# ysong1231/SimRank

Hardware: AMD Instinct MI355X
Metric: simrank_iterations_per_sec (higher is better)
Workload: dtype f32

## Files before the change

### simrank_amd/csrc/api.hip

```cpp
#include <algorithm>
#include <chrono>
#include <cstring>
#include <mutex>
#include <unordered_map>
#include <string>
#include <thread>
#include <vector>

#include "common.h"

namespace simrank {

static thread_local char g_err[512] = "";

void set_error(const char* fmt, ...) {
    va_list ap;
    va_start(ap, fmt);
    vsnprintf(g_err, sizeof(g_err), fmt, ap);
    va_end(ap);
}

Tuning& tuning() {
    static Tuning t;
    return t;
// ... 747 lines not shown
extern "C" {

int simrank_graph_destroy(simrank_graph* g) {
    if (!g) return SIMRANK_OK;
    plan_free(g->rowptr);
    plan_free(g->col);
    plan_free(g->col16);
    plan_free(g->rowscale);
    plan_free(g->t_rowptr);
    plan_free(g->t_col);
    plan_free(g->t_pos);
    plan_free(g->ev_hubidx);
    plan_free(g->ev_hub_image);
#ifndef SIMRANK_HOST_ONLY
    if (g->ev_hub_ready) (void)hipEventDestroy((hipEvent_t)g->ev_hub_ready);
#endif
    plan_free(g->tile_row0);
    plan_free(g->sym_map);
    free_dense_plan(g->dense);
    free_fused_plan(g->fused);
#ifdef SIMRANK_EXPERIMENT_FUSED2
    free_fused2_plan(g->fused2);
#endif
    delete g;
    return SIMRANK_OK;
}

int simrank_graph_set_dense_terms(simrank_graph* g, int32_t terms) {
    SR_REQUIRE(g, "graph is NULL");
    SR_REQUIRE(terms == 1 || terms == 3, "dense terms must be 3 (exact) or 1 (fp16 operand)");
    g->tun.dense_terms = terms;
    return SIMRANK_OK;
}

int simrank_graph_shape(const simrank_graph* g, int64_t* n_rows, int64_t* n_cols, int64_t* nnz) {
    SR_REQUIRE(g, "graph is NULL");
    if (n_rows) *n_rows = g->n_rows;
    if (n_cols) *n_cols = g->n_cols;
    if (nnz) *nnz = g->nnz;
    return SIMRANK_OK;
}

int simrank_set_tuning(const char* key, int64_t value) {
    SR_REQUIRE(key, "key is NULL");
    std::lock_guard<std::mutex> lock(tuning_mutex());
    Tuning& t = tuning();
    if (!strcmp(key, "panel")) {
        SR_REQUIRE(value == 0 || value == 16 || value == 32 || value == 64 || value == 128 ||
                       value == 256,
                   "panel must be 0, 16, 32, 64, 128 or 256");
        t.panel = value;
    } else if (!strcmp(key, "xcd_map")) {
        t.xcd_map = value ? 1 : 0;
    } else if (!strcmp(key, "tile")) {
        SR_REQUIRE(value == 0 || value == 16 || value == 32 || value == 64, "tile must be 0, 16, 32 or 64");
        t.tile = value;
    } else if (!strcmp(key, "huge")) {
        SR_REQUIRE(value >= 64 && value <= (1 << 30), "huge must be >= 64");
        t.huge = value;
    } else if (!strcmp(key, "triangle")) {
        t.triangle = value ? 1 : 0;
    } else if (!strcmp(key, "stream_nt")) {
        t.stream_nt = value ? 1 : 0;
    } else if (!strcmp(key, "balance")) {
        SR_REQUIRE(value >= 0 && value <= 1024, "balance must be 0 (uniform tiles) .. 1024");
        t.balance = value;
    } else if (!strcmp(key, "dense_min")) {
        SR_REQUIRE(value >= 0 && value <= 128, "dense_min must be 0 (off) .. 128");
        t.dense_min = value;
    } else if (!strcmp(key, "probe_mask")) {
        SR_REQUIRE(value < 0 || getenv("SIMRANK_ENABLE_PROBES"),
                   "probe knobs give WRONG results (measurement only): set SIMRANK_ENABLE_PROBES=1 to use them");
        t.probe_mask = value < 0 ? -1 : value;
    } else if (!strcmp(key, "dense_terms")) {
        SR_REQUIRE(value == 1 || value == 3, "dense_terms must be 3 (exact) or 1 (fp16 operand)");
        t.dense_terms = value;
    } else if (!strcmp(key, "probe_flags")) {
        SR_REQUIRE(value == 0 || getenv("SIMRANK_ENABLE_PROBES"),
                   "probe knobs give WRONG results (measurement only): set SIMRANK_ENABLE_PROBES=1 to use them");
        t.probe_flags = value & 63;
    } else if (!strcmp(key, "addr32")) {
        t.addr32 = value ? 1 : 0;
    } else if (!strcmp(key, "lean")) {
        SR_REQUIRE(value == 0 || value == 1, "lean must be 0 or 1");
        t.lean = value;
    } else if (!strcmp(key, "ids16")) {
        t.ids16 = value ? 1 : 0;
    } else if (!strcmp(key, "sym_desc")) {
        t.sym_desc = value ? 1 : 0;
    } else if (!strcmp(key, "dense_sym")) {
        t.dense_sym = value < 0 ? -1 : (value ? 1 : 0);
    } else if (!strcmp(key, "fuse")) {
#ifdef SIMRANK_EXPERIMENT_FUSED2
        SR_REQUIRE(value >= 0 && value <= 2, "fuse must be 0 (two launches), 1 (one launch) or 2 (one persistent launch)");
#else
        SR_REQUIRE(value == 0 || value == 1, "fuse must be 0 (two launches) or 1 (one launch)");
#endif
        t.fuse = value;
    } else if (!strcmp(key, "ev_hub")) {
        SR_REQUIRE(value >= 0 && value <= 1000, "ev_hub must be 0 (off) .. 1000 (thousandths of the row count)");
        t.ev_hub = value;
    } else if (!strcmp(key, "fuse_min")) {
        SR_REQUIRE(value == 0 || (value >= 2 && value <= 128), "fuse_min must be 2 .. 128, or 0 (quads that pay)");
        t.fuse_min = value;
    } else if (!strcmp(key, "fuse_pays")) {
        SR_REQUIRE(value >= -1 && value <= 8192, "fuse_pays must be -1 (automatic) .. 8192");
        t.fuse_pays = value;
    } else if (!strcmp(key, "fuse_unit")) {
        SR_REQUIRE(value >= 4 && value <= (1 << 20), "fuse_unit must be >= 4");
        t.fuse_unit = value;
    } else if (!strcmp(key, "fuse_store")) {
        SR_REQUIRE(value >= 0 && value <= 3, "fuse_store must be 0 .. 3");
        t.fuse_store = value;
    } else if (!strcmp(key, "fuse_meta_nt")) {
        t.fuse_meta_nt = value ? 1 : 0;
    } else if (!strcmp(key, "fuse_order")) {
        SR_REQUIRE(value >= 0 && value <= 64, "fuse_order must be 0 .. 64");
        t.fuse_order = value;
    } else if (!strcmp(key, "fuse_max_rows")) {
        SR_REQUIRE(value >= 0, "fuse_max_rows must be >= 0");
        t.fuse_max_rows = value;
    } else if (!strcmp(key, "fuse_rows")) {
        SR_REQUIRE(value >= 64 && value <= (int64_t(1) << 40), "fuse_rows must be >= 64");
        t.fuse_rows = value;
    } else if (!strcmp(key, "ev_tri")) {
        t.ev_tri = value ? 1 : 0;
    } else if (!strcmp(key, "fuse_shards")) {
        t.fuse_shards = value ? 1 : 0;
    } else if (!strcmp(key, "fuse_cap")) {
        SR_REQUIRE(value >= 1000 && value <= (int64_t(1) << 40), "fuse_cap must be >= 1000");
        t.fuse_cap = value;
    } else if (!strcmp(key, "fuse_wgs")) {
        SR_REQUIRE(value >= 1 && value <= 8, "fuse_wgs must be 1 .. 8");
        t.fuse_wgs = value;
    } else if (!strcmp(key, "fuse_group")) {
        SR_REQUIRE(value >= 1 && value <= 4, "fuse_group must be 1 .. 4");
        t.fuse_group = value;
    } else if (!strcmp(key, "fuse_sym")) {
        SR_REQUIRE(value >= -1 && value <= 1, "fuse_sym must be -1 (automatic), 0 or 1");
        t.fuse_sym = value;
    } else if (!strcmp(key, "fuse_steps")) {
        SR_REQUIRE(value >= -1 && value <= (1 << 20), "fuse_steps must be >= 0, or -1 (by the operand's size)");
        t.fuse_steps = value;
    } else if (!strcmp(key, "fuse_dens")) {
        SR_REQUIRE(value >= 0 && value <= (1 << 20), "fuse_dens must be >= 0");
        t.fuse_dens = value;
    } else if (!strcmp(key, "dense_cols")) {
        SR_REQUIRE(value >= 1 && value <= (1 << 20), "dense_cols must be >= 1");
        t.dense_cols = value;
    } else if (!strcmp(key, "restrict_support")) {
        SR_REQUIRE(value >= -1 && value <= 1, "restrict_support must be -1 (automatic), 0 or 1");
        t.restrict_support = value;
    } else if (!strcmp(key, "leg1_skip")) {
        t.leg1_skip = value ? 1 : 0;
    } else if (!strcmp(key, "leg1_order")) {
        SR_REQUIRE(value >= -1 && value <= 1, "leg1_order must be -1 (by the graph's size), 0 or 1");
        t.leg1_order = value;
    } else {
        SR_REQUIRE(false, "unknown tuning key '%s'", key);
    }
    return SIMRANK_OK;
}

int simrank_get_tuning(const char* key, int64_t* value) {
    SR_REQUIRE(key && value, "NULL argument");
    const Tuning t = tuning_snapshot();
    if (!strcmp(key, "panel")) *value = t.panel;
    else if (!strcmp(key, "xcd_map")) *value = t.xcd_map;
    else if (!strcmp(key, "stream_nt")) *value = t.stream_nt;
    else if (!strcmp(key, "tile")) *value = t.tile;
    else if (!strcmp(key, "triangle")) *value = t.triangle;
    else if (!strcmp(key, "huge")) *value = t.huge;
    else if (!strcmp(key, "balance")) *value = t.balance;
    else if (!strcmp(key, "dense_min")) *value = t.dense_min;
    else if (!strcmp(key, "dense_cols")) *value = t.dense_cols;
    else if (!strcmp(key, "dense_sym")) *value = t.dense_sym;
    else if (!strcmp(key, "fuse")) *value = t.fuse;
    else if (!strcmp(key, "ev_hub")) *value = t.ev_hub;
    else if (!strcmp(key, "fuse_min")) *value = t.fuse_min;
    else if (!strcmp(key, "fuse_pays")) *value = t.fuse_pays;
    else if (!strcmp(key, "fuse_steps")) *value = t.fuse_steps;
    else if (!strcmp(key, "fuse_dens")) *value = t.fuse_dens;
    else if (!strcmp(key, "fuse_unit")) *value = t.fuse_unit;
    else if (!strcmp(key, "fuse_group")) *value = t.fuse_group;
    else if (!strcmp(key, "fuse_sym")) *value = t.fuse_sym;
    else if (!strcmp(key, "fuse_cap")) *value = t.fuse_cap;
    else if (!strcmp(key, "fuse_shards")) *value = t.fuse_shards;
    else if (!strcmp(key, "ev_tri")) *value = t.ev_tri;
    else if (!strcmp(key, "fuse_rows")) *value = t.fuse_rows;
    else if (!strcmp(key, "fuse_wgs")) *value = t.fuse_wgs;
    else if (!strcmp(key, "fuse_max_rows")) *value = t.fuse_max_rows;
    else if (!strcmp(key, "fuse_order")) *value = t.fuse_order;
    else if (!strcmp(key, "fuse_store")) *value = t.fuse_store;
    else if (!strcmp(key, "fuse_meta_nt")) *value = t.fuse_meta_nt;
    else if (!strcmp(key, "sym_desc")) *value = t.sym_desc;
    else if (!strcmp(key, "ids16")) *value = t.ids16;
    else if (!strcmp(key, "lean")) *value = t.lean;
    else if (!strcmp(key, "addr32")) *value = t.addr32;
    else if (!strcmp(key, "probe_flags")) *value = t.probe_flags;
    else if (!strcmp(key, "dense_terms")) *value = t.dense_terms;
    else if (!strcmp(key, "probe_mask")) *value = t.probe_mask;
    else if (!strcmp(key, "restrict_support")) *value = t.restrict_support;
    else if (!strcmp(key, "leg1_skip")) *value = t.leg1_skip;
    else if (!strcmp(key, "leg1_order")) *value = t.leg1_order;
    else SR_REQUIRE(false, "unknown tuning key '%s'", key);
    return SIMRANK_OK;
}

int simrank_graph_get(const simrank_graph* g, const char* key, int64_t* value) {
    SR_REQUIRE(g && key && value, "NULL argument");
    if (!strcmp(key, "fused_ids16")) *value = g->fused ? g->fused->ids16 : -1;
    else if (!strcmp(key, "gather_ids16")) *value = (g->col16 && g->tun.ids16) ? 1 : 0;
    else SR_REQUIRE(false, "unknown graph key '%s'", key);
    return SIMRANK_OK;
}

}
```

### simrank_amd/csrc/common.h

```cpp
#pragma once
#include <hip/hip_runtime.h>

#include <cstdarg>
#include <atomic>
#include <cstdint>
#include <cstdio>
#include <cstdlib>
#include <cstring>
#include <functional>
#include <vector>

#include "simrank_hip.h"

namespace simrank {

void set_error(const char* fmt, ...);

#define SR_HIP(call)                                                                   \
    do {                                                                               \
        hipError_t e_ = (call);                                                        \
        if (e_ != hipSuccess) {                                                        \
            ::simrank::set_error("%s failed: %s (%s:%d)", #call, hipGetErrorString(e_), \
                                 __FILE__, __LINE__);                                  \
            return SIMRANK_ERR_HIP;                                                    \
        }                                                                              \
    } while (0)

#define SR_REQUIRE(cond, ...)                 \
    do {                                      \
        if (!(cond)) {                        \
            ::simrank::set_error(__VA_ARGS__); \
            return SIMRANK_ERR_INVALID;       \
        }                                     \
    } while (0)

struct Tuning {
    int64_t panel = 0;
    int64_t xcd_map = 1;
    int64_t stream_nt = 1;
    int64_t tile = 0;
    int64_t huge = 512;
    int64_t triangle = 1;
    int64_t balance = 2;
    int64_t dense_min = 4;
    int64_t dense_cols = 128;
    int64_t dense_terms = 3;
    int64_t probe_mask = -1;
    int64_t probe_flags = 0;
    int64_t addr32 = 1;
    int64_t lean = 1;
    int64_t ids16 = 1;
    int64_t sym_desc = 1;
    int64_t ev_tri = 1;
    int64_t ev_hub = 14;
    int64_t fuse = 1;
    int64_t fuse_min = 0;
    int64_t fuse_pays = -1;
    int64_t fuse_steps = -1;
    int64_t fuse_dens = 0;
    int64_t fuse_unit = 48;
    int64_t fuse_rows = 8192;
    int64_t fuse_store = 1;
    int64_t fuse_meta_nt = 0;
    int64_t fuse_order = 0;
    int64_t fuse_max_rows = 1 << 20;
    int64_t fuse_cap = 40000;
    int64_t fuse_wgs = 4;
    int64_t fuse_shards = 1;
    int64_t fuse_group = 3;
    int64_t fuse_sym = -1;
    int64_t leg1_skip = 1;
    int64_t leg1_order = -1;
    int64_t dense_lazy = 0;
    int64_t dense_sym = -1;
    int64_t restrict_support = -1;
};
inline int32_t restrict_choice(const Tuning& t, int64_t live, int64_t total) {
    return t.restrict_support < 0 ? (2 * live < total ? 1 : 0) : int32_t(t.restrict_support != 0);
}
Tuning& tuning();
Tuning tuning_snapshot();


#ifdef SIMRANK_HOST_ONLY
inline hipError_t plan_alloc(void** p, size_t bytes) {
    *p = malloc(bytes ? bytes : 1);
    return *p ? hipSuccess : hipErrorOutOfMemory;
}
inline hipError_t plan_upload(void* d, const void* h, size_t bytes) { memcpy(d, h, bytes); return hipSuccess; }
inline hipError_t plan_download(void* h, const void* d, size_t bytes) { memcpy(h, d, bytes); return hipSuccess; }
inline void plan_free(void* p) { free(p); }
#else
int pool_alloc(void** dptr, size_t bytes);
int pool_free(void* ptr);
inline hipError_t plan_alloc(void** p, size_t bytes) {
    const int rc = pool_alloc(p, bytes);
    return rc == SIMRANK_OK ? hipSuccess : (rc == SIMRANK_ERR_ALLOC ? hipErrorOutOfMemory : hipErrorUnknown);
}
inline hipError_t plan_upload(void* d, const void* h, size_t bytes) { return hipMemcpy(d, h, bytes, hipMemcpyHostToDevice); }
inline hipError_t plan_download(void* h, const void* d, size_t bytes) { return hipMemcpy(h, d, bytes, hipMemcpyDeviceToHost); }
inline void plan_free(void* p) { (void)pool_free(p); }
#endif

int graph_create_with(const Tuning& tun, int64_t n_rows, int64_t n_cols, int64_t nnz, const int32_t* rowptr,
                      const int32_t* col, const float* rowscale, simrank_graph** out,
                      const std::function<int(simrank_graph*)>* after_base = nullptr);

int pool_alloc(void** dptr, size_t bytes);
int pool_free(void* ptr);
void pool_trim(int device);
void pool_stats(int device, int64_t* cached_bytes, int64_t* cached_blocks, int64_t* limit_bytes);
void handback_release_slabs(int device);
int rows_to_host(const void* S, int64_t rows_pad, int64_t n, const int32_t* inv_dev, const int32_t* rows, int32_t n_rows,
                 float* dst, int64_t ld, int elem, float scale, hipStream_t stream);
inline hipError_t pool_hip_alloc(void** p, size_t bytes) {
    const int rc = pool_alloc(p, bytes);
    return rc == SIMRANK_OK ? hipSuccess : (rc == SIMRANK_ERR_ALLOC ? hipErrorOutOfMemory : hipErrorUnknown);
}

int identity_leg1_blocked(const simrank_graph* g, float* Tt, int64_t t_rows_pad, void* stream);
int identity_leg1_blocked_h16(const simrank_graph* g, uint16_t* Tt, int64_t t_rows_pad, float scale, void* stream);

struct PlanPrep {
    std::vector<int32_t> ord, inv;
    std::vector<int32_t> rp, cl;
    std::vector<float> rs;
    bool asym = false;
    std::vector<int32_t> first_block;
};
constexpr int32_t kLeg1Never = 0x7FFFFFFF;
void first_block_table(int64_t n, const int32_t* rp, const int32_t* cl, std::vector<int32_t>& first_block);
struct BiPlanPrep {
    std::vector<int32_t> rowptr21, col21;
    std::vector<int32_t> ord[2], inv[2];
    std::vector<int32_t> rp[2], cl[2];
    std::vector<float> rs[2];
    bool asym = false;
};
int plan_prepare(int64_t n, int64_t nnz, const int32_t* rowptr, const int32_t* col, const float* rowscale,
                 const simrank_plan_options* opt, PlanPrep* out);
int shard_prepare(int64_t n, int64_t nnz, const int32_t* rowptr, const int32_t* col, const float* rowscale,
                  const float* apriori, int64_t ld_apriori, bool reorder, int32_t deal, PlanPrep* out, bool allow_asym = false);
int shard_biplan_prepare(int64_t n1, int64_t n2, int64_t nnz, const int32_t* rowptr12, const int32_t* col12,
                         const float* rowscale1, const float* rowscale2, const simrank_biplan_options* opt, int32_t deal1,
                         int32_t deal2, BiPlanPrep* out, bool allow_asym = false);
bool prior_symmetric(const float* a, int64_t ld, int64_t n);
int biplan_prepare(int64_t n1, int64_t n2, int64_t nnz, const int32_t* rowptr12, const int32_t* col12,
                   const float* rowscale1, const float* rowscale2, const simrank_biplan_options* opt, BiPlanPrep* out);

inline int64_t fuse_min_steps(const Tuning& t, int64_t K) {
    return t.fuse_steps >= 0 ? t.fuse_steps : (K * 128 > (int64_t(4) << 20) ? 8 : 20);
}

constexpr int64_t kSpeculateBelow = 16384;

inline hipStream_t as_stream(void* s) { return reinterpret_cast<hipStream_t>(s); }
inline bool aligned16(const void* p) { return (reinterpret_cast<uintptr_t>(p) & 15u) == 0; }

}


struct simrank_dense_plan {
    int32_t n_units = 0;
    int32_t n_slabs = 0;
    int32_t n_blocks_dense = 0;
    int64_t total_k = 0;
    int64_t nnz_covered = 0;
    int32_t* unit_row0 = nullptr;
    int32_t* unit_slab = nullptr;
    int32_t* unit_kofs = nullptr;
    int32_t* dcols = nullptr;
    uint4* afrag = nullptr;
    int32_t* block_slab0 = nullptr;
    int32_t* block_nslab = nullptr;
    int64_t r_nnz = 0;
    int32_t r_max_row = 0;
    int32_t* r_rowptr = nullptr;
    int32_t* r_col = nullptr;
    uint16_t* r_col16 = nullptr;
    int32_t* r_tile_row0 = nullptr;
    int32_t r_n_tiles = 0;
    int32_t* r_sym_map = nullptr;
    int32_t r_sym_blocks = 0;
    float* part = nullptr;
    size_t part_cap = 0;
};

struct simrank_fused_plan {
    int32_t n_units = 0;
    int32_t n_blocks = 0;
    int32_t ids16 = 0;
    int64_t n_quads = 0;
    int64_t n_steps = 0;
    int64_t nnz_covered = 0;
    int64_t r_nnz = 0;
    int32_t* units = nullptr;
    int32_t n_pslots = 0, n_cslots = 0;
    float* partials = nullptr;
    int32_t* tickets = nullptr;
    int32_t cap_panels = 0;
    uint16_t* dcols16 = nullptr;
    int32_t* dcols32 = nullptr;
    uint4* abits = nullptr;
    int2* gmeta = nullptr;
    uint16_t* sids16 = nullptr;
    int32_t* sids32 = nullptr;
    std::vector<int32_t> unit_last;
};

#ifdef SIMRANK_EXPERIMENT_FUSED2
struct simrank_fused2_plan {
    int32_t n_items = 0;
    int32_t n_blocks = 0;
    int32_t ids16 = 0;
    int32_t cap_panels = 0;
    int64_t n_quads = 0, n_steps = 0, nnz_covered = 0, r_nnz = 0;
    int32_t* items = nullptr;
    int32_t n_pslots = 0, n_cslots = 0;
    float* partials = nullptr;
    int32_t* tickets = nullptr;
    uint32_t* heads = nullptr;
    uint16_t* dcols16 = nullptr;
    int32_t* dcols32 = nullptr;
    uint4* abits = nullptr;
    int2* gmeta = nullptr;
    uint16_t* sids16 = nullptr;
    int32_t* sids32 = nullptr;
};
#endif

namespace simrank {
constexpr int kFB = 128;
constexpr int kSub = 4;
void free_fused_plan(simrank_fused_plan* p);
int build_fused_plan(simrank_graph* g, const int32_t* rowptr, const int32_t* col, const float* rowscale);
int launch_fused_trans(const simrank_graph* g, const float* X, int64_t x_rows_pad, int64_t L, float* Y,
                       int64_t y_rows_pad, hipStream_t st, const int32_t* first_block = nullptr);
void fused_leg1_counts(const simrank_graph* g, int64_t L, const int32_t* first_block_host, int64_t* units, int64_t* skipped);
int spmm_blocked_is_triangle(const simrank_graph* g, const float* X, int64_t x_rows_pad, int64_t n_cols_x, float* Y,
                             int64_t y_rows_pad, const simrank_epilogue* ep, bool* triangle);
int spmm_blocked_leg1(const simrank_graph* g, const float* X, int64_t x_rows_pad, int64_t n_cols_x, float* Y,
                      int64_t y_rows_pad, const int32_t* first_block, bool* skipping, void* stream);
bool fused_sym_applies(const simrank_graph* g, int64_t x_rows_pad, int64_t L, int64_t y_rows_pad);
int launch_fused_sym(const simrank_graph* g, const float* X, int64_t x_rows_pad, int64_t L, float* Y, int64_t y_rows_pad,
                     float coef, float lbd, double eps, const uint8_t* ev, const float* ap, const float* prev,
                     unsigned long long* n_changed, int32_t set_diag, int32_t count_any, hipStream_t st);
bool fused_rowmajor_fits(const simrank_graph* g, const float* X, int64_t ldx, int64_t L, const float* Y, int64_t t_block,
                         int64_t t_pad);
int launch_fused_trans_rowmajor(const simrank_graph* g, const float* X, int64_t ldx, int64_t L, float* Y, int64_t t_block,
                                int64_t t_pad, hipStream_t st);
#ifdef SIMRANK_EXPERIMENT_FUSED2
void free_fused2_plan(simrank_fused2_plan* p);
int build_fused2_plan(simrank_graph* g, const int32_t* rowptr, const int32_t* col, const float* rowscale);
int launch_fused2_trans(const simrank_graph* g, const float* X, int64_t x_rows_pad, int64_t L, float* Y,
                        int64_t y_rows_pad, hipStream_t st);
#endif
struct DenseUse {
    const float* part = nullptr;
    int64_t ldp = 0;
    const int32_t* block_slab0 = nullptr;
    const int32_t* block_nslab = nullptr;
};
void free_dense_plan(simrank_dense_plan* p);
int build_dense_plan(simrank_graph* g, const int32_t* rowptr, const int32_t* col);
int launch_dense_tiles(const simrank_graph* g, const float* X, int64_t ldx, int64_t L, bool tri,
                       hipStream_t st, DenseUse* use);
int64_t build_tiles(const int32_t* rowptr, int64_t n_rows, int64_t nnz, int64_t balance,
                    std::vector<int32_t>& tile_row0, std::vector<int32_t>& sym_map, bool sym_descending);
}

struct simrank_graph {
    int64_t n_rows = 0, n_cols = 0, nnz = 0;
    int32_t* rowptr = nullptr;
    int32_t* col = nullptr;
    uint16_t* col16 = nullptr;
    float* rowscale = nullptr;
    int32_t* t_rowptr = nullptr;
    int32_t* t_col = nullptr;
    int32_t* t_pos = nullptr;
    int32_t* ev_hubidx = nullptr;
    int32_t ev_hubs = 0;
    uint8_t* ev_hub_image = nullptr;
    void* ev_hub_ready = nullptr;
    int32_t max_row_nnz = 0;
    int32_t* tile_row0 = nullptr;
    int32_t n_tiles = 0;
    int32_t* sym_map = nullptr;
    int32_t sym_blocks = 0;
    simrank_dense_plan* dense = nullptr;
    simrank_fused_plan* fused = nullptr;
    std::atomic<int> fused_build{0};
#ifdef SIMRANK_EXPERIMENT_FUSED2
    simrank_fused2_plan* fused2 = nullptr;
#endif
    simrank::Tuning tun;
};
```

### simrank_amd/csrc/fused.hip

```cpp
#include <algorithm>
#include <cstring>
#include <numeric>
#include <vector>

#include <cstdlib>

#include <mutex>
#include <thread>

#include "common.h"
#include "fused_dev.h"

namespace simrank {

constexpr int kTS = 132;
#ifndef SIMRANK_KMINUNITS
#define SIMRANK_KMINUNITS 64
#endif
#ifndef SIMRANK_KGROUPENTRIES
#define SIMRANK_KGROUPENTRIES 6144
#endif
#ifndef SIMRANK_KMAXREM
#define SIMRANK_KMAXREM 256
#endif
constexpr int kMinUnits = SIMRANK_KMINUNITS;
constexpr int kGroupEntries = SIMRANK_KGROUPENTRIES;
constexpr int64_t kPaysGatherBound = 192, kPaysMfmaBound = 256, kStepInEntries = 77;
constexpr int kMaxRem = SIMRANK_KMAXREM;

struct FusedArgs {
    const float* X;
    float* Y;
    int64_t x_rows_pad, y_rows_pad;
    int64_t L, M;
    int64_t x_panel_stride;
    uint32_t x_pitch;
    int32_t x_bytes;
    int32_t y_chunked;
    int64_t t_block, t_pad;
    int32_t n_panels, n_units, nt;
    int32_t x_sentinel;
    int32_t idx_mask;
    int32_t meta_nt;
    int32_t probe;
    const float* rowscale;
    const int32_t* units;
    float* partials;
    int32_t* tickets;
    int32_t n_pslots, n_cslots;
    const uint16_t* dcols16;
    const int32_t* dcols32;
    const uint4* abits;
    const int2* gmeta;
    const uint16_t* sids16;
    const int32_t* sids32;
    float coef, lbd;
    double eps;
    const uint8_t* ev;
    const float* ap;
    const float* prev;
    unsigned long long* n_changed;
    int32_t set_diag, count_any;
    const int32_t* first_block;
};

#ifndef SIMRANK_HOST_ONLY
#if defined(__HIP_DEVICE_COMPILE__) && !defined(__gfx942__) && !defined(__gfx950__)
#error "fused.hip: the sc1 hand-off between the units of a split block is written for gfx942 / gfx950"
#endif
#ifdef SIMRANK_FUSED_STAMPS
constexpr int kFstCap = 1 << 15;
__device__ unsigned long long g_fst[kFstCap * 8];
__device__ unsigned int g_fst_base;
__device__ __forceinline__ unsigned long long fst_now() {
    unsigned long long t;
    __builtin_amdgcn_sched_barrier(0);
    asm volatile("s_memtime %0\n\ts_waitcnt lgkmcnt(0)" : "=s"(t) :: "memory");
    __builtin_amdgcn_sched_barrier(0);
    return t;
}
#define FST(i)                                                                              \
    do {                                                                                    \
        const unsigned long long now_ = fst_now();                                          \
        if (threadIdx.x == 0 && blockIdx.x - g_fst_base < unsigned(kFstCap))                \
            g_fst[size_t(blockIdx.x - g_fst_base) * 8 + (i)] = now_;                        \
    } while (0)
#else
#define FST(i) do {} while (0)
#endif

#ifndef SIMRANK_FUSED_LB
#define SIMRANK_FUSED_LB 4
#endif
#ifndef SIMRANK_FUSED_LB_SYM
#define SIMRANK_FUSED_LB_SYM 3
#endif
template <bool IDS16, bool SYM = false>
__global__ __launch_bounds__(256, SYM ? SIMRANK_FUSED_LB_SYM : SIMRANK_FUSED_LB) void fused_trans_kernel(const FusedArgs p) {
    __shared__ __attribute__((aligned(16))) float tile[32 * kTS];
    __shared__ __attribute__((aligned(16))) float bbuf_all[4 * 16 * 32];
    __shared__ __attribute__((aligned(16))) uint4 lut[256];
    __shared__ __attribute__((aligned(16))) int2 gm_lds[kSub * 4 * 8 * 4];

    const int lane = threadIdx.x & 63;
    const int wave = __builtin_amdgcn_readfirstlane(threadIdx.x >> 6);
    const uint32_t bid = blockIdx.x;
    const uint32_t local = bid >> 3;
    const int panel = int(local / uint32_t(p.n_units)) * 8 + int(bid & 7);
    if (panel >= p.n_panels) return;
    const uint32_t unit = local % uint32_t(p.n_units);
    const int32_t* un = p.units + size_t(unit) * 32;
    FST(0);
#ifdef SIMRANK_FUSED_STAMPS
    if (threadIdx.x == 0 && blockIdx.x - g_fst_base < unsigned(kFstCap)) {
        const unsigned xcc = __builtin_amdgcn_s_getreg((4 - 1) << 11 | 0 << 6 | 20);
        const unsigned hw = __builtin_amdgcn_s_getreg((16 - 1) << 11 | 0 << 6 | 4);
        g_fst[size_t(blockIdx.x - g_fst_base) * 8 + 5] = (unsigned long long)xcc << 32 | hw;
        g_fst[size_t(blockIdx.x - g_fst_base) * 8 + 6] = (unsigned long long)panel << 32 | unit;
    }
#endif
    const int b0 = un[0];
    const int64_t c0 = int64_t(panel) * 32;
    const int n_sub_all = un[8];
    const int n_sub_sym = SYM ? min(n_sub_all, int((c0 + 31) >> 7) - b0 + 1) : n_sub_all;
    if (SYM && n_sub_sym <= 0) return;
    if constexpr (!SYM) {
        if (p.first_block && b0 + n_sub_all - 1 < p.first_block[panel]) return;
    }
    const int g = lane >> 3, q = lane & 7, gbase = lane & ~7;
    const uint32_t qoff = uint32_t(q) * 16u;

    const float* xbase = p.X + int64_t(panel) * p.x_panel_stride;
    const __amdgpu_buffer_rsrc_t srd = __builtin_amdgcn_make_buffer_rsrc(
        const_cast<float*>(xbase), 0, p.x_bytes - (p.x_pitch == 128u ? 0 : panel * 128), 0x00020000);
    const uint32_t pitch = p.x_pitch;
    const int sent = p.x_sentinel;

    const int quad0 = un[1];
    const int nq = (p.probe & 4) ? 0 : un[2];
    const int unit_k = un[3], unit_nb = un[4], pslot = un[5], cslot = un[6];
    const bool has_set = !(p.probe & 4) && un[7] != 0;
    const int n_sub = n_sub_sym;
    const int per = (nq + 3) >> 2;
    const int n_active = per ? (nq + per - 1) / per : 0;

    const int q_lo = wave * per, q_hi = min(nq, q_lo + per);
    auto ld_ids = [&](int qd) -> int {
        const size_t at = size_t(quad0 + qd) * 64 + lane;
        if constexpr (IDS16) return int(p.dcols16[at]) & p.idx_mask;
        else return p.dcols32[at] & p.idx_mask;
    };
    const int qa0 = max(0, min(q_lo, nq - 1)), qa1 = max(0, min(q_lo + 1, q_hi - 1));
    int ids_a = ld_ids(qa0);
    uint4 aw_a = p.abits[size_t(quad0 + qa0) * 64 + lane];
    int ids_b = ld_ids(qa1);
    uint4 aw_b = p.abits[size_t(quad0 + qa1) * 64 + lane];

    const int32_t* wm = un + 9 + wave * 5;
    const int round0 = wm[0];
    const int e1 = wm[1], e2 = wm[2], e3 = wm[3], e4 = wm[4];
    const int n_rounds = (p.probe & 1) ? 0 : (n_sub == 1 ? e1 : n_sub == 2 ? e2 : n_sub == 3 ? e3 : e4);
    auto fix_sid = [&](int v) -> int {
        if constexpr (IDS16) return v == 0xFFFF ? sent : (v & p.idx_mask);
        else return v < 0 ? sent : (v & p.idx_mask);
    };
    auto ld_sid_raw = [&](int r) -> int {
        const size_t at = (size_t(round0) + size_t(min(r, max(n_rounds - 1, 0)))) * 64 + lane;
        if constexpr (IDS16) return p.meta_nt ? int(__builtin_nontemporal_load(p.sids16 + at)) : int(p.sids16[at]);
        else return p.meta_nt ? __builtin_nontemporal_load(p.sids32 + at) : p.sids32[at];
    };
    auto ld_sid = [&](int r) -> int { return fix_sid(ld_sid_raw(r)); };
    int iv0 = sent, iv1 = sent;
    {
        const int sbA = q >> 2, sbB = 2 + (q >> 2);
        const int2* src = p.gmeta + ((size_t(un[29]) * 4 + wave) * 8 + g) * 4 + (q & 3);
        int2* dst = gm_lds + (wave * 8 + g) * 4 + (q & 3);
        int2 a = src[size_t(min(sbA, n_sub - 1)) * 4 * 8 * 4];
        int2 c = src[size_t(min(sbB, n_sub - 1)) * 4 * 8 * 4];
        int raw0 = 0, raw1 = 0;
        if (n_rounds > 0) {
            raw0 = ld_sid_raw(0);
            raw1 = ld_sid_raw(1);
        }
        __builtin_amdgcn_sched_barrier(0);
        if (sbA >= n_sub) a = make_int2(int(0xFFFFFFFFu), 0);
        if (sbB >= n_sub) c = make_int2(int(0xFFFFFFFFu), 0);
        dst[sbA * 4 * 8 * 4] = a;
        dst[sbB * 4 * 8 * 4] = c;
        if (n_rounds > 0) {
            iv0 = fix_sid(raw0);
            iv1 = fix_sid(raw1);
        }
    }

    float4 rA0 = make_float4(0.f, 0.f, 0.f, 0.f), rA1 = rA0, rB0 = rA0, rB1 = rA0;
    auto issue = [&](int ids, int s4, float4& x0, float4& x1) {
        x0 = ld_seg_p(srd, __shfl(ids, s4 * 16 + g), pitch, qoff);
        x1 = ld_seg_p(srd, __shfl(ids, s4 * 16 + 8 + g), pitch, qoff);
    };
    if (q_lo < q_hi) {
        issue(ids_a, 0, rA0, rA1);
        issue(ids_a, 1, rB0, rB1);
    }

    FST(1);
    if (nq > 0) {
        {
            const unsigned e = threadIdx.x;
            uint4 v;
            v.x = ((e >> 0) & 1u) * 0x3F80u | ((e >> 1) & 1u) * 0x3F800000u;
            v.y = ((e >> 2) & 1u) * 0x3F80u | ((e >> 3) & 1u) * 0x3F800000u;
            v.z = ((e >> 4) & 1u) * 0x3F80u | ((e >> 5) & 1u) * 0x3F800000u;
            v.w = ((e >> 6) & 1u) * 0x3F80u | ((e >> 7) & 1u) * 0x3F800000u;
            lut[e] = v;
        }
        __syncthreads();
        f32x16 acc[4];
#pragma unroll
        for (int t = 0; t < 4; ++t)
#pragma unroll
            for (int i = 0; i < 16; ++i) acc[t][i] = 0.f;
        if (q_lo < q_hi) {
            float* bbuf = bbuf_all + wave * (16 * 32);
            const int n = lane & 31, h = lane >> 5;
            struct Terms { uint32_t lo[4], mid[4], hi[4]; };
            auto stage = [&](const float4& x0, const float4& x1, float (&x)[8]) {
                wave_lds_order();
                *reinterpret_cast<float4*>(bbuf + g * 32 + q * 4) = x0;
                *reinterpret_cast<float4*>(bbuf + (8 + g) * 32 + q * 4) = x1;
                wave_lds_order();
#pragma unroll
                for (int j = 0; j < 8; ++j) x[j] = bbuf[(8 * h + j) * 32 + n];
            };
            auto split = [&](const float (&x)[8], Terms& t) {
#pragma unroll
                for (int j = 0; j < 4; ++j) split3f(x[2 * j], x[2 * j + 1], t.hi[j], t.mid[j], t.lo[j]);
            };
            auto mma = [&](const Terms& t, uint32_t aw) {
                const bf16x8 bl = frag(t.lo[0], t.lo[1], t.lo[2], t.lo[3]);
                const bf16x8 bm = frag(t.mid[0], t.mid[1], t.mid[2], t.mid[3]);
                const bf16x8 bh = frag(t.hi[0], t.hi[1], t.hi[2], t.hi[3]);
#pragma unroll
                for (int tt = 0; tt < 4; ++tt) {
                    const bf16x8 a = __builtin_bit_cast(bf16x8, lut[(aw >> (8 * tt)) & 255u]);
                    acc[tt] = __builtin_amdgcn_mfma_f32_32x32x16_bf16(a, bl, acc[tt], 0, 0, 0);
                    acc[tt] = __builtin_amdgcn_mfma_f32_32x32x16_bf16(a, bm, acc[tt], 0, 0, 0);
                    acc[tt] = __builtin_amdgcn_mfma_f32_32x32x16_bf16(a, bh, acc[tt], 0, 0, 0);
                }
            };
            Terms tA, tB;
            float x[8];
            stage(rA0, rA1, x);
            split(x, tA);
            issue(ids_a, 2, rA0, rA1);
            for (int qd = q_lo; qd < q_hi; ++qd) {
                stage(rB0, rB1, x);
                issue(ids_a, 3, rB0, rB1);
                mma(tA, aw_a.x);
                split(x, tB);
                stage(rA0, rA1, x);
                issue(ids_b, 0, rA0, rA1);
                mma(tB, aw_a.y);
                split(x, tA);
                stage(rB0, rB1, x);
                issue(ids_b, 1, rB0, rB1);
                mma(tA, aw_a.z);
                split(x, tB);
                stage(rA0, rA1, x);
                issue(ids_b, 2, rA0, rA1);
                mma(tB, aw_a.w);
                split(x, tA);
                ids_a = ids_b;
                aw_a = aw_b;
                const int nx = min(qd + 2, q_hi - 1);
                ids_b = ld_ids(nx);
                aw_b = p.abits[size_t(quad0 + nx) * 64 + lane];
            }
        }
        {
            const int n = lane & 31, h = lane >> 5;
            for (int w = 0; w < n_active; ++w) {
                if (wave == w) {
#pragma unroll
                    for (int t = 0; t < 4; ++t)
#pragma unroll
                        for (int i4 = 0; i4 < 4; ++i4) {
                            float4* dst = reinterpret_cast<float4*>(tile + n * kTS + 32 * t + 8 * i4 + 4 * h);
                            float4 v = make_float4(acc[t][4 * i4], acc[t][4 * i4 + 1], acc[t][4 * i4 + 2], acc[t][4 * i4 + 3]);
                            if (w > 0) {
                                const float4 o = *dst;
                                v.x += o.x; v.y += o.y; v.z += o.z; v.w += o.w;
                            }
                            *dst = v;
                        }
                }
                __syncthreads();
            }
        }
    }
    const bool split_unit = un[30] != 0;
    if (split_unit && nq == 0) {
        for (int x4 = threadIdx.x; x4 < 32 * kTS / 4; x4 += 256)
            reinterpret_cast<float4*>(tile)[x4] = make_float4(0.f, 0.f, 0.f, 0.f);
        __syncthreads();
    }
    const bool has_d = has_set || split_unit;
    unsigned changed = 0;
    const unsigned slot = ((blockIdx.x * 4u + unsigned(wave)) * 7u) % SIMRANK_CHANGED_SLOTS;
    bool check_prev = false;
    if constexpr (SYM) {
        check_prev = p.prev != nullptr;
        if (check_prev && p.count_any) check_prev = __hip_atomic_load(p.n_changed + slot, __ATOMIC_RELAXED, __HIP_MEMORY_SCOPE_AGENT) == 0;
        check_prev = __builtin_amdgcn_readfirstlane(int(check_prev)) != 0;
    }

    FST(2);
    {
        int sb = 0;
        int r_base = 0;
        auto end_of = [&](int k) __attribute__((always_inline)) -> int { return k == 0 ? e1 : k == 1 ? e2 : k == 2 ? e3 : e4; };
        int r_end = (p.probe & 1) ? 0 : e1;
        const int2* gmp = gm_lds + (wave * 8 + g) * 4;
        wave_lds_order();
        auto unpack = [](const int2& m) __attribute__((always_inline)) -> int3 {
            const unsigned u = unsigned(m.x);
            const int row = int(u & 255u), end = int(u >> 8);
            return make_int3(row == 255 ? -1 : row, m.y, end == 0xFFFFFF ? -1 : end);
        };
        int3 m_cur = unpack(gmp[0]);
        float4 cur = make_float4(0.f, 0.f, 0.f, 0.f);
        int krow = 0;
        auto emit = [&](const int3& m, const float4& sv) __attribute__((always_inline)) {
            if (m.x >= 0) {
                const float sc = split_unit ? 1.0f : __int_as_float(m.y);
                float* tp = tile + (4 * q) * kTS + m.x;
                const float d0 = has_d ? tp[0] : 0.f, d1 = has_d ? tp[kTS] : 0.f;
                const float d2 = has_d ? tp[2 * kTS] : 0.f, d3 = has_d ? tp[3 * kTS] : 0.f;
                tp[0] = (sv.x + d0) * sc;
                tp[kTS] = (sv.y + d1) * sc;
                tp[2 * kTS] = (sv.z + d2) * sc;
                tp[3 * kTS] = (sv.w + d3) * sc;
            }
        };
        auto row_end = [&](int f) __attribute__((always_inline)) {
            if (f + 1 == m_cur.z) {
                emit(m_cur, cur);
                cur = make_float4(0.f, 0.f, 0.f, 0.f);
                ++krow;
                m_cur = unpack(gmp[sb * 128 + min(krow, 3)]);
                if (krow > 3) m_cur.z = -1;
            }
        };
        auto finish = [&]() __attribute__((always_inline)) {
            for (int k = krow; k < 4; ++k) emit(unpack(gmp[sb * 128 + k]), make_float4(0.f, 0.f, 0.f, 0.f));
            FST(3);
            __syncthreads();
            const int row0 = (b0 + sb) * kFB;
            if (unit_nb > 1) {
                typedef unsigned v4u __attribute__((ext_vector_type(4)));
                float* mine = p.partials + (size_t(pslot) * p.n_panels + panel) * (32 * kFB);
                const __amdgpu_buffer_rsrc_t msrd = __builtin_amdgcn_make_buffer_rsrc(mine, 0, 32 * kFB * 4, 0x00020000);
#pragma unroll
                for (int it = 0; it < 4; ++it) {
                    const int x = threadIdx.x + it * 256;
                    const int c = x >> 5, r4 = (x & 31) * 4;
                    const float4 v = *reinterpret_cast<const float4*>(tile + c * kTS + r4);
                    v4u o;
                    o.x = __float_as_uint(v.x); o.y = __float_as_uint(v.y); o.z = __float_as_uint(v.z); o.w = __float_as_uint(v.w);
                    __builtin_amdgcn_raw_buffer_store_b128(o, msrd, (c * kFB + r4) * 4, 0, 16);
                }
                asm volatile("s_waitcnt vmcnt(0)" ::: "memory");
                __syncthreads();
                int* flag = reinterpret_cast<int*>(bbuf_all);
                if (threadIdx.x == 0) {
                    int* tk = p.tickets + size_t(cslot) * p.n_panels + panel;
                    const int t = __hip_atomic_fetch_add(tk, 1, __ATOMIC_RELAXED, __HIP_MEMORY_SCOPE_AGENT);
                    const int last = t == unit_nb - 1;
                    if (last) __hip_atomic_store(tk, 0, __ATOMIC_RELAXED, __HIP_MEMORY_SCOPE_AGENT);
                    *flag = last;
                }
                __syncthreads();
                if (!*flag) {
                    sb = n_sub;
                    return;
                }
                const int first = pslot - unit_k;
                float4 acc4[4];
                auto piece = [&](int k, int it) -> float4 {
                    const int x = threadIdx.x + it * 256;
                    const int c = x >> 5, r4 = (x & 31) * 4;
                    const float* src = p.partials + (size_t(first + k) * p.n_panels + panel) * (32 * kFB);
                    const __amdgpu_buffer_rsrc_t ssrd =
                        __builtin_amdgcn_make_buffer_rsrc(const_cast<float*>(src), 0, 32 * kFB * 4, 0x00020000);
                    const v4u w = __builtin_amdgcn_raw_buffer_load_b128(ssrd, (c * kFB + r4) * 4, 0, 16);
                    return make_float4(__uint_as_float(w.x), __uint_as_float(w.y), __uint_as_float(w.z), __uint_as_float(w.w));
                };
                for (int k = 0; k < unit_nb; ++k) {
                    float4 va[4];
#pragma unroll
                    for (int it = 0; it < 4; ++it) va[it] = piece(k, it);
#pragma unroll
                    for (int it = 0; it < 4; ++it) {
                        if (k == 0) acc4[it] = va[it];
                        else { acc4[it].x += va[it].x; acc4[it].y += va[it].y; acc4[it].z += va[it].z; acc4[it].w += va[it].w; }
                    }
                }
#pragma unroll
                for (int it = 0; it < 4; ++it) {
                    const int x = threadIdx.x + it * 256;
                    const int c = x >> 5, r4 = (x & 31) * 4;
                    float scv[4];
#pragma unroll
                    for (int j = 0; j < 4; ++j) scv[j] = row0 + r4 + j < p.M ? p.rowscale[row0 + r4 + j] : 0.f;
                    float4 a4 = acc4[it];
                    a4.x *= scv[0]; a4.y *= scv[1]; a4.z *= scv[2]; a4.w *= scv[3];
                    *reinterpret_cast<float4*>(tile + c * kTS + r4) = a4;
                }
                __syncthreads();
            }
            const int nrows = int(min(int64_t(kFB), p.M - row0));
            const int rows_out = max(0, min(32, nrows - 32 * wave));
            const int cols_here = int(min(int64_t(32), p.L - c0));
            bool mirror = true;
            if constexpr (SYM) {
                const int64_t rt_row0 = int64_t(row0) + 32 * wave;
                const bool on_diag = c0 == rt_row0;
                mirror = c0 > rt_row0;
                if (rows_out > 0 && (mirror || on_diag)) {
                    typedef unsigned v4u __attribute__((ext_vector_type(4)));
                    const int64_t pbase = int64_t(panel) * p.y_rows_pad;
                    const int bytes_f = int(p.y_rows_pad * 128);
                    const __amdgpu_buffer_rsrc_t ysrd2 = __builtin_amdgcn_make_buffer_rsrc(p.Y + pbase * 32, 0, bytes_f, 0x00020000);
                    const __amdgpu_buffer_rsrc_t osrd = __builtin_amdgcn_make_buffer_rsrc(
                        const_cast<float*>(p.prev ? p.prev + pbase * 32 : p.Y), 0, p.prev ? bytes_f : 0, 0x00020000);
                    const __amdgpu_buffer_rsrc_t asrd = __builtin_amdgcn_make_buffer_rsrc(
                        const_cast<float*>(p.ap ? p.ap + pbase * 32 : p.Y), 0, p.ap ? bytes_f : 0, 0x00020000);
                    const __amdgpu_buffer_rsrc_t esrd = __builtin_amdgcn_make_buffer_rsrc(
                        const_cast<uint8_t*>(p.ev ? p.ev + pbase * 32 : reinterpret_cast<const uint8_t*>(p.Y)), 0,
                        p.ev ? int(p.y_rows_pad * 32) : 0, 0x00020000);
                    const int nvalid = max(0, min(4, cols_here - 4 * q));
                    const float keep = 1.0f - p.lbd;
#pragma unroll
                    for (int half = 0; half < 2; ++half) {
                    unsigned w_ev[2];
                    v4u w_ap[2], w_old[2];
#pragma unroll
                    for (int it = 0; it < 2; ++it) {
                        const int rr = 8 * (2 * half + it) + g;
                        const uint32_t a = uint32_t(rt_row0 + rr);
                        const bool on = rr < rows_out;
                        const uint32_t row = on ? a : 0x7FFFFF0u;
                        w_ev[it] = __builtin_amdgcn_raw_buffer_load_b32(esrd, int(row * 32u + 4u * q), 0, 2);
                        w_ap[it] = __builtin_amdgcn_raw_buffer_load_b128(asrd, int(row * 128u + qoff), 0, 2);
                        w_old[it] = check_prev ? __builtin_amdgcn_raw_buffer_load_b128(osrd, int(row * 128u + qoff), 0, 2)
                                               : v4u{0u, 0u, 0u, 0u};
                    }
#pragma unroll
                    for (int it = 0; it < 2; ++it) {
                        const int rr = 8 * (2 * half + it) + g;
                        if (rr < rows_out) {
                            const int64_t a = rt_row0 + rr;
                            float* tp = tile + (4 * q) * kTS + 32 * wave + rr;
                            float o[4] = {tp[0] * p.coef, tp[kTS] * p.coef, tp[2 * kTS] * p.coef, tp[3 * kTS] * p.coef};
                            if (p.ev) {
                                const unsigned w = w_ev[it];
                                o[0] *= 1.0f - __builtin_ldexpf(1.0f, -int(w & 255u));
                                o[1] *= 1.0f - __builtin_ldexpf(1.0f, -int((w >> 8) & 255u));
                                o[2] *= 1.0f - __builtin_ldexpf(1.0f, -int((w >> 16) & 255u));
                                o[3] *= 1.0f - __builtin_ldexpf(1.0f, -int(w >> 24));
                            }
                            if (p.ap) {
                                const float pr[4] = {__uint_as_float(w_ap[it].x), __uint_as_float(w_ap[it].y),
                                                     __uint_as_float(w_ap[it].z), __uint_as_float(w_ap[it].w)};
#pragma unroll
                                for (int i = 0; i < 4; ++i) o[i] = keep * o[i] + p.lbd * pr[i];
                            }
                            if (p.set_diag) {
                                const int64_t d = a - (c0 + 4 * q);
#pragma unroll
                                for (int i = 0; i < 4; ++i)
                                    if (d == i) o[i] = 1.0f;
                            }
                            if (check_prev) {
                                const float old[4] = {__uint_as_float(w_old[it].x), __uint_as_float(w_old[it].y),
                                                      __uint_as_float(w_old[it].z), __uint_as_float(w_old[it].w)};
#pragma unroll
                                for (int i = 0; i < 4; ++i)
                                    changed += (i < nvalid && fabs(double(o[i]) - double(old[i])) > p.eps) ? (mirror ? 2u : 1u) : 0u;
                            }
                            tp[0] = o[0]; tp[kTS] = o[1]; tp[2 * kTS] = o[2]; tp[3 * kTS] = o[3];
                            if (!(p.probe & 2)) {
                                const int yoff = int(uint32_t(a) * 128u + qoff);
                                if (nvalid == 4) {
                                    v4u out;
                                    out.x = __float_as_uint(o[0]); out.y = __float_as_uint(o[1]);
                                    out.z = __float_as_uint(o[2]); out.w = __float_as_uint(o[3]);
                                    if (p.nt) __builtin_amdgcn_raw_buffer_store_b128(out, ysrd2, yoff, 0, 2);
                                    else __builtin_amdgcn_raw_buffer_store_b128(out, ysrd2, yoff, 0, 0);
                                } else {
#pragma unroll
                                    for (int i = 0; i < 4; ++i)
                                        if (i < nvalid) __builtin_amdgcn_raw_buffer_store_b32(__float_as_uint(o[i]), ysrd2, yoff + 4 * i, 0, 0);
                                }
                            }
                        }
                    }
                    }
                    wave_lds_order();
                }
            }
            if (rows_out > 0 && mirror && !(p.probe & 2)) {
                int cstride = 32;
                float* base = p.Y + ((int64_t(row0 >> 5) + wave) * p.y_rows_pad + c0) * 32;
                if (p.y_chunked) {
                    const int64_t h = row0 / p.t_block;
                    const int64_t rows_h = min(p.t_block, p.M - h * p.t_block);
                    cstride = int(rows_h + p.t_pad);
                    base = p.Y + h * p.L * (p.t_block + p.t_pad) + c0 * cstride + (row0 - h * p.t_block) + 32 * wave;
                }
                const float* tw = tile + 32 * wave;
                const __amdgpu_buffer_rsrc_t ysrd =
                    __builtin_amdgcn_make_buffer_rsrc(base, 0, (31 * cstride + 32) * 4, 0x00020000);
                if ((rows_out & 3) == 0) {
#pragma unroll
                    for (int it = 0; it < 4; ++it) {
                        const int x = lane + it * 64;
                        const int c = x >> 3;
                        const int r4 = (x & 7) * 4;
                        if (c < cols_here && r4 < rows_out) {
                            const float4 v = *reinterpret_cast<const float4*>(tw + c * kTS + r4);
                            typedef unsigned v4u __attribute__((ext_vector_type(4)));
                            v4u o;
                            o.x = __float_as_uint(v.x); o.y = __float_as_uint(v.y);
                            o.z = __float_as_uint(v.z); o.w = __float_as_uint(v.w);
                            const int off = (c * cstride + r4) * 4;
                            switch (p.nt) {
                                case 0: __builtin_amdgcn_raw_buffer_store_b128(o, ysrd, off, 0, 0); break;
                                case 1: __builtin_amdgcn_raw_buffer_store_b128(o, ysrd, off, 0, 2); break;
                                case 2: __builtin_amdgcn_raw_buffer_store_b128(o, ysrd, off, 0, 16); break;
                                default: __builtin_amdgcn_raw_buffer_store_b128(o, ysrd, off, 0, 17); break;
                            }
                        }
                    }
                } else {
                    for (int x = lane; x < 32 * 32; x += 64) {
                        const int c = x >> 5, r = x & 31;
                        if (c < cols_here && r < rows_out) base[c * cstride + r] = tw[c * kTS + r];
                    }
                }
            }
            ++sb;
            if (sb < n_sub) {
                __syncthreads();
                r_base = r_end;
                r_end = (p.probe & 1) ? 0 : end_of(sb);
                krow = 0;
                cur = make_float4(0.f, 0.f, 0.f, 0.f);
                m_cur = unpack(gmp[sb * 128]);
            }
        };
        auto issue8 = [&](int iv, float4 (&v)[8]) {
#pragma unroll
            for (int j = 0; j < 8; ++j) v[j] = ld_seg_p(srd, __shfl(iv, gbase + j), pitch, qoff);
        };
        auto consume = [&](const float4 (&v)[8], int r) {
#pragma unroll
            for (int j = 0; j < 8; ++j) {
                cur.x += v[j].x; cur.y += v[j].y; cur.z += v[j].z; cur.w += v[j].w;
                row_end(8 * (r - r_base) + j);
            }
            while (sb < n_sub && r + 1 == r_end) finish();
        };
        while (sb < n_sub && r_end == r_base) finish();
        if (n_rounds > 0) {
            float4 vA[8], vB[8];
            issue8(iv0, vA);
            int r = 0;
            while (r + 2 < n_rounds) {
                const int iv2 = ld_sid(r + 2);
                issue8(iv1, vB);
                consume(vA, r);
                iv1 = ld_sid(r + 3);
                issue8(iv2, vA);
                consume(vB, r + 1);
                r += 2;
            }
            if (r + 1 < n_rounds) {
                issue8(iv1, vB);
                consume(vA, r);
                consume(vB, r + 1);
            } else {
                consume(vA, r);
            }
        }
        while (sb < n_sub) finish();
    }
    if constexpr (SYM) {
        if (p.prev) {
#pragma unroll
            for (int off = 32; off > 0; off >>= 1) changed += __shfl_down(changed, off);
            if (lane == 0 && changed) atomicAdd(p.n_changed + slot, (unsigned long long)changed);
        }
    }
    FST(4);
}

#endif

template <typename T>
static int upload_vec(T** d, const std::vector<T>& h) {
    const size_t bytes = std::max<size_t>(16, h.size() * sizeof(T));
    SR_HIP(plan_alloc((void**)d, bytes));
    if (!h.empty()) SR_HIP(plan_upload(*d, h.data(), h.size() * sizeof(T)));
    return SIMRANK_OK;
}

void free_fused_plan(simrank_fused_plan* p) {
    if (!p) return;
    plan_free(p->units);
#ifndef SIMRANK_HOST_ONLY
    (void)pool_free(p->partials); (void)pool_free(p->tickets);
#endif
    plan_free(p->dcols16); plan_free(p->dcols32); plan_free(p->abits);
    plan_free(p->gmeta); plan_free(p->sids16); plan_free(p->sids32);
    delete p;
}

int build_fused_plan(simrank_graph* g, const int32_t* rowptr, const int32_t* col, const float* rowscale) {
    const int64_t M = g->n_rows, K = g->n_cols;
    const bool by_quads = g->tun.fuse_min == 0;
    const int64_t thr = std::max<int64_t>(2, g->tun.fuse_min);
    const int64_t min_steps = fuse_min_steps(g->tun, g->n_cols);
    const int64_t nblk = (M + kFB - 1) / kFB;
    int64_t pays = g->tun.fuse_pays;
    if (by_quads && pays < 0) {
        pays = kPaysGatherBound;
        std::vector<uint16_t> cnt(size_t(K), 0);
        std::vector<int32_t> touched;
        std::vector<int32_t> hist(size_t(kFB) + 1);
        int64_t s_steps = 0, s_rem = 0;
        const int64_t stride = std::max<int64_t>(1, nblk / 16);
        for (int64_t b = 0; b < nblk; b += stride) {
            const int64_t lo = b * kFB, hi = std::min<int64_t>(M, lo + kFB);
            touched.clear();
            std::fill(hist.begin(), hist.end(), 0);
            for (int32_t j = rowptr[lo]; j < rowptr[hi]; ++j)
                if (cnt[col[j]]++ == 0) touched.push_back(col[j]);
            for (int32_t c : touched) { ++hist[cnt[c]]; cnt[c] = 0; }
            int64_t nq = 0, cov = 0, in_quad = 0, gain = 0;
            bool open = true;
            for (int c = kFB; c >= 1 && open; --c) {
                int64_t left = hist[size_t(c)];
                while (left > 0) {
                    const int64_t take = std::min<int64_t>(left, 64 - in_quad);
                    in_quad += take; gain += take * c; left -= take;
                    if (in_quad == 64) {
                        if (gain < pays) { open = false; in_quad = 0; gain = 0; break; }
                        ++nq; cov += gain; in_quad = 0; gain = 0;
                    }
                }
            }
            if (open && in_quad > 0 && gain >= pays) { ++nq; cov += gain; }
            if (4 * nq < min_steps) { nq = 0; cov = 0; }
            s_steps += 4 * nq;
            s_rem += int64_t(rowptr[hi] - rowptr[lo]) - cov;
        }
        if (kStepInEntries * s_steps > s_rem) pays = kPaysMfmaBound;
    }
    const bool ids16 = K <= 65535 && g->tun.ids16;
    std::vector<int32_t> blk_quad0(size_t(nblk) + 1, 0);
    std::vector<int32_t> dcols;
    std::vector<uint32_t> abits;
    std::vector<std::vector<int32_t>> blk_sids((size_t(nblk) + size_t(kSub)) * 4);
    std::vector<int32_t> blk_gmeta((size_t(nblk) + size_t(kSub)) * 32 * 4 * 2, int32_t(0xFFFFFFFFu));
    std::fill(blk_gmeta.begin(), blk_gmeta.begin() + size_t(nblk) * 32 * 4 * 2, 0);
    std::vector<int64_t> cost(size_t(nblk), 0), blk_rem(size_t(nblk), 0);
    std::vector<int32_t> blk_ng(size_t(nblk), 0), blk_gslot(size_t(nblk), 0);
    size_t extra_gm = 0;
    int64_t covered = 0, steps_total = 0, r_nnz = 0;
    struct GatherOut { std::vector<int32_t> sids[4]; int32_t gmeta[32 * 4 * 2]; };
    struct BlockOut {
        std::vector<int32_t> dcols;
        std::vector<uint32_t> abits;
        int32_t nq = 0, U = 0, ng = 0;
        int64_t covered = 0, rem = 0, cost = 0;
        std::vector<GatherOut> gus;
    };
    struct Scratch {
        std::vector<uint16_t> cnt;
        std::vector<int32_t> kpos, touched, set;
        std::vector<int32_t> rem[kFB];
        explicit Scratch(int64_t K) : cnt(size_t(K), 0), kpos(size_t(K), -1) {}
    };
    auto process_block = [&](int64_t b, Scratch& sc, BlockOut& out) {
        std::vector<uint16_t>& cnt = sc.cnt;
        std::vector<int32_t>& kpos = sc.kpos;
        std::vector<int32_t>& touched = sc.touched;
        std::vector<int32_t>& set = sc.set;
        std::vector<int32_t>* rem = sc.rem;
        const int64_t lo = b * kFB, hi = std::min<int64_t>(M, lo + kFB);
        touched.clear();
        set.clear();
        for (int32_t j = rowptr[lo]; j < rowptr[hi]; ++j)
            if (cnt[col[j]]++ == 0) touched.push_back(col[j]);
        if (by_quads) {
            std::stable_sort(touched.begin(), touched.end(), [&](int32_t x, int32_t y) { return cnt[x] > cnt[y]; });
            size_t n = 0;
            while (n < touched.size()) {
                const size_t e = std::min(touched.size(), n + 64);
                int64_t gain = 0;
                for (size_t i = n; i < e; ++i) gain += cnt[touched[i]];
                if (gain < pays) break;
                n = e;
            }
            for (size_t i = 0; i < n; ++i) { set.push_back(touched[i]); kpos[touched[i]] = 0; }
        } else {
            for (int32_t c : touched)
                if (cnt[c] >= thr) { set.push_back(c); kpos[c] = 0; }
        }
        {
            const int64_t steps = (int64_t)(set.size() + 15) / 16;
            bool keep = steps >= min_steps;
            if (!keep && g->tun.fuse_dens > 0 && steps >= 4) {
                int64_t cov = 0;
                for (int32_t c : set) cov += cnt[c];
                keep = cov >= g->tun.fuse_dens * steps;
            }
            if (!keep) {
                for (int32_t c : set) kpos[c] = -1;
                set.clear();
// ... 107 lines not shown
            Scratch sc(K);
            for (int64_t b = 0; b < nblk; ++b) process_block(b, sc, outs[(size_t)b]);
        } else {
            std::vector<std::thread> th;
            int64_t b0 = 0;
            for (int t = 0; t < n_thr; ++t) {
                int64_t b1 = nblk;
                if (t + 1 < n_thr) {
                    const int64_t target = int64_t(rowptr[M]) * (t + 1) / n_thr;
                    b1 = b0;
                    while (b1 < nblk && rowptr[std::min<int64_t>(M, b1 * kFB)] < target) ++b1;
                }
                th.emplace_back([&, b0, b1]() {
                    Scratch sc(K);
                    for (int64_t b = b0; b < b1; ++b) process_block(b, sc, outs[(size_t)b]);
                });
                b0 = b1;
            }
            for (std::thread& x : th) x.join();
        }
    }
    for (int64_t b = 0; b < nblk; ++b) {
        BlockOut& o = outs[(size_t)b];
        blk_quad0[size_t(b) + 1] = blk_quad0[size_t(b)] + o.nq;
        steps_total += (o.U + 15) / 16;
        dcols.insert(dcols.end(), o.dcols.begin(), o.dcols.end());
        abits.insert(abits.end(), o.abits.begin(), o.abits.end());
        covered += o.covered;
        r_nnz += o.rem;
        blk_rem[size_t(b)] = o.rem;
        blk_ng[size_t(b)] = o.ng;
        cost[size_t(b)] = o.cost;
        for (size_t gu = 0; gu < o.gus.size(); ++gu) {
            const size_t slot = gu == 0 ? size_t(b) : size_t(nblk) + size_t(kSub) + extra_gm++;
            if (gu > 0) {
                blk_gmeta.resize((slot + 1) * 32 * 4 * 2, 0);
                blk_sids.resize((slot + 1) * 4);
            }
            if (gu == 1) blk_gslot[size_t(b)] = (int32_t)slot;
            std::copy(o.gus[gu].gmeta, o.gus[gu].gmeta + 32 * 4 * 2, blk_gmeta.begin() + slot * 32 * 4 * 2);
            for (int w = 0; w < 4; ++w) blk_sids[slot * 4 + size_t(w)].swap(o.gus[gu].sids[w]);
        }
        o = BlockOut();
    }
    const int64_t unit_q = std::max<int64_t>(4, g->tun.fuse_unit);
    struct Unit { int32_t b0, nsub, q0, nq, k, nb; int64_t cost; int32_t gslot, split; };
    std::vector<Unit> ulist;
    for (int64_t group = std::min<int64_t>(kSub, std::max<int64_t>(1, g->tun.fuse_group));; group /= 2) {
        ulist.clear();
        for (int64_t b = 0; b < nblk;) {
            const int32_t q0 = blk_quad0[size_t(b)], nqb = blk_quad0[size_t(b) + 1] - q0;
            if (blk_ng[size_t(b)] > 0) {
                const int32_t n_m = nqb > 0 ? (int32_t)std::max<int64_t>(1, (nqb + unit_q - 1) / unit_q) : 0;
                const int32_t n_g = blk_ng[size_t(b)], nb = n_m + n_g;
                for (int32_t k = 0; k < n_m; ++k) {
                    const int32_t lo = (int32_t)(int64_t(nqb) * k / n_m), hi = (int32_t)(int64_t(nqb) * (k + 1) / n_m);
                    ulist.push_back({(int32_t)b, 1, q0 + lo, hi - lo, k, nb, cost[size_t(b)], (int32_t)nblk, 1});
                }
                for (int32_t k = 0; k < n_g; ++k)
                    ulist.push_back({(int32_t)b, 1, q0, 0, n_m + k, nb, cost[size_t(b)],
                                     k == 0 ? (int32_t)b : blk_gslot[size_t(b)] + (k - 1), 1});
                ++b;
            } else if (nqb > 0) {
                ulist.push_back({(int32_t)b, 1, q0, nqb, 0, 1, cost[size_t(b)], (int32_t)b, 0});
                ++b;
            } else {
                int64_t e = b + 1, c = cost[size_t(b)], entries = blk_rem[size_t(b)];
                while (e < nblk && e - b < group && blk_quad0[size_t(e) + 1] == blk_quad0[size_t(e)] && blk_ng[size_t(e)] == 0 &&
                       entries + blk_rem[size_t(e)] <= kGroupEntries) {
                    entries += blk_rem[size_t(e)];
                    c += cost[size_t(e++)];
                }
                ulist.push_back({(int32_t)b, (int32_t)(e - b), q0, 0, 0, 1, c, (int32_t)b, 0});
                b = e;
            }
        }
        if (group <= 1 || (int64_t)ulist.size() >= kMinUnits) break;
    }
    std::stable_sort(ulist.begin(), ulist.end(), [](const Unit& x, const Unit& y) {
        return x.cost != y.cost ? x.cost > y.cost : (x.b0 != y.b0 ? x.b0 < y.b0 : x.k < y.k);
    });
    if (g->tun.fuse_order > 0 && ulist.size() > 8) {
        std::vector<Unit> heavy, light, mixed;
        for (const Unit& u : ulist) ((u.nq > 0 || u.split) ? heavy : light).push_back(u);
        const size_t span = std::max(heavy.size(), std::min(ulist.size(), ulist.size() / size_t(g->tun.fuse_order)));
        size_t hi = 0, li = 0;
        for (size_t pos = 0; pos < ulist.size(); ++pos) {
            const bool want_heavy = hi < heavy.size() && (li >= light.size() || hi * span <= pos * heavy.size());
            if (want_heavy) mixed.push_back(heavy[hi++]);
            else mixed.push_back(light[li++]);
        }
        ulist.swap(mixed);
    }
    std::vector<int32_t> units(ulist.size() * 32, 0), sids;
    blk_gmeta.resize(blk_gmeta.size() + size_t(kSub) * 32 * 4 * 2, int32_t(0xFFFFFFFFu));
    sids.reserve(size_t(r_nnz) + ulist.size() * 512);
    int32_t n_pslots = 0, n_cslots = 0;
    std::vector<int32_t> blk_pslot(size_t(nblk), -1), blk_cslot(size_t(nblk), -1);
    for (size_t i = 0; i < ulist.size(); ++i) {
        const Unit& u = ulist[i];
        int32_t* rec = &units[i * 32];
        rec[0] = u.b0; rec[1] = u.q0; rec[2] = u.nq; rec[3] = u.k; rec[4] = u.nb;
        rec[5] = -1; rec[6] = -1;
        rec[7] = u.nq > 0 ? 1 : 0;
        rec[8] = u.nsub;
        rec[29] = u.gslot;
        rec[30] = u.split;
        if (u.nb > 1) {
            if (blk_pslot[size_t(u.b0)] < 0) {
                blk_pslot[size_t(u.b0)] = n_pslots;
                blk_cslot[size_t(u.b0)] = n_cslots;
                n_pslots += u.nb;
                ++n_cslots;
            }
            rec[5] = blk_pslot[size_t(u.b0)] + u.k;
            rec[6] = blk_cslot[size_t(u.b0)];
        }
        for (int w = 0; w < 4; ++w) {
            int32_t* wm = rec + 9 + w * 5;
            wm[0] = (int32_t)(sids.size() / 64);
            int32_t rounds = 0;
            for (int sb = 0; sb < kSub; ++sb) {
                if (sb < u.nsub) {
                    const std::vector<int32_t>& bs = blk_sids[size_t(u.gslot + sb) * 4 + size_t(w)];
                    sids.insert(sids.end(), bs.begin(), bs.end());
                    rounds += (int32_t)(bs.size() / 64);
                }
                wm[1 + sb] = rounds;
            }
        }
    }

    if (const char* dump = std::getenv("SIMRANK_DUMP_FUSED_PLAN")) {
        if (FILE* f = std::fopen(dump, "wb")) {
            const int64_t hdr[8] = {0x53524450, M, K, (int64_t)(units.size() / 32), (int64_t)(sids.size() / 64),
                                    (int64_t)(dcols.size() / 64), r_nnz, covered};
            std::fwrite(hdr, sizeof(int64_t), 8, f);
            std::fwrite(units.data(), sizeof(int32_t), units.size(), f);
            std::fwrite(sids.data(), sizeof(int32_t), sids.size(), f);
            std::fwrite(dcols.data(), sizeof(int32_t), dcols.size(), f);
            std::fclose(f);
        }
    }
    simrank_fused_plan* pl = new simrank_fused_plan;
    pl->n_units = (int32_t)(units.size() / 32);
    pl->n_blocks = (int32_t)nblk;
    pl->n_pslots = n_pslots;
    pl->n_cslots = n_cslots;
    pl->n_quads = blk_quad0[size_t(nblk)];
    pl->n_steps = steps_total;
    pl->nnz_covered = covered;
    pl->r_nnz = r_nnz;
    pl->ids16 = ids16 ? 1 : 0;
    pl->unit_last.reserve(ulist.size());
    for (const Unit& u : ulist) pl->unit_last.push_back(u.b0 + u.nsub - 1);
    std::sort(pl->unit_last.begin(), pl->unit_last.end());
    dcols.resize(dcols.size() + 64, 0);
    abits.resize(abits.size() + 64 * 4, 0u);
    int rc = upload_vec(&pl->units, units);
    if (!rc) {
        if (ids16) {
            std::vector<uint16_t> d16(dcols.begin(), dcols.end());
            rc = upload_vec(&pl->dcols16, d16);
        } else {
            rc = upload_vec(&pl->dcols32, dcols);
        }
    }
    if (!rc) rc = upload_vec(reinterpret_cast<uint32_t**>(&pl->abits), abits);
    if (!rc) rc = upload_vec(reinterpret_cast<int32_t**>(&pl->gmeta), blk_gmeta);
    if (!rc) {
        if (ids16) {
            std::vector<uint16_t> s16(sids.size());
            for (size_t i = 0; i < sids.size(); ++i) s16[i] = sids[i] < 0 ? uint16_t(0xFFFF) : uint16_t(sids[i]);
            rc = upload_vec(&pl->sids16, s16);
        } else {
            rc = upload_vec(&pl->sids32, sids);
        }
    }
#ifndef SIMRANK_HOST_ONLY
    if (!rc && n_pslots > 0) {
        const int32_t panels = (int32_t)((std::max<int64_t>(M, K) + 31) / 32);
        hipError_t e = pool_hip_alloc((void**)&pl->partials, size_t(n_pslots) * panels * 32 * kFB * sizeof(float));
        if (e == hipSuccess) e = pool_hip_alloc((void**)&pl->tickets, size_t(n_cslots) * panels * sizeof(int32_t));
        if (e == hipSuccess) e = hipMemset(pl->tickets, 0, size_t(n_cslots) * panels * sizeof(int32_t));
        if (e != hipSuccess) {
            set_error("one-launch plan: partial sums of %d split blocks: %s", n_cslots, hipGetErrorString(e));
            (void)hipGetLastError();
            rc = e == hipErrorOutOfMemory ? SIMRANK_ERR_ALLOC : SIMRANK_ERR_HIP;
        } else {
            pl->cap_panels = panels;
        }
    }
#endif
    if (rc) {
        free_fused_plan(pl);
        return rc;
    }
    g->fused = pl;
    return SIMRANK_OK;
}

static int launch_fused(const simrank_graph* g, FusedArgs& a, hipStream_t st, bool sym = false) {
    simrank_fused_plan* pl = g->fused;
    static std::mutex launch_mutex;
    std::lock_guard<std::mutex> launch_lock(launch_mutex);
    a.M = g->n_rows;
    a.n_panels = int32_t((a.L + 31) / 32);
    a.n_units = pl->n_units;
    a.nt = (int32_t)(g->tun.stream_nt ? g->tun.fuse_store : 0);
    a.probe = (int32_t)g->tun.probe_flags;
    a.meta_nt = (int32_t)g->tun.fuse_meta_nt;
    a.idx_mask = (int32_t)g->tun.probe_mask;
    a.units = pl->units;
    a.rowscale = g->rowscale;
    if (pl->n_pslots > 0 && a.n_panels > pl->cap_panels) {
        SR_HIP(hipStreamSynchronize(st));
        (void)pool_free(pl->partials); (void)pool_free(pl->tickets);
        pl->partials = nullptr; pl->tickets = nullptr; pl->cap_panels = 0;
        SR_HIP(pool_hip_alloc((void**)&pl->partials, size_t(pl->n_pslots) * a.n_panels * 32 * kFB * sizeof(float)));
        SR_HIP(pool_hip_alloc((void**)&pl->tickets, size_t(pl->n_cslots) * a.n_panels * sizeof(int32_t)));
        SR_HIP(hipMemsetAsync(pl->tickets, 0, size_t(pl->n_cslots) * a.n_panels * sizeof(int32_t), st));
        pl->cap_panels = a.n_panels;
    }
    a.partials = pl->partials; a.tickets = pl->tickets;
    a.n_pslots = pl->n_pslots; a.n_cslots = pl->n_cslots;
    a.dcols16 = pl->dcols16; a.dcols32 = pl->dcols32; a.abits = pl->abits;
    a.gmeta = pl->gmeta; a.sids16 = pl->sids16; a.sids32 = pl->sids32;
    const int64_t grid = int64_t((a.n_panels + 7) / 8) * 8 * a.n_units;
    SR_REQUIRE(grid > 0 && grid < (int64_t(1) << 31), "grid of %lld blocks", (long long)grid);
#ifdef SIMRANK_FUSED_STAMPS
    static const unsigned lds_pad = getenv("SIMRANK_FUSED_PAD") ? (unsigned)atoi(getenv("SIMRANK_FUSED_PAD")) : 0u;
    {
        const char* e = getenv("SIMRANK_FST_BASE");
        const unsigned base = e ? (unsigned)atoll(e) : 0u;
        SR_HIP(hipMemcpyToSymbolAsync(HIP_SYMBOL(g_fst_base), &base, sizeof(base), 0, hipMemcpyHostToDevice, st));
    }
#else
    const unsigned lds_pad = 0;
#endif
#ifdef SIMRANK_HOST_ONLY
    (void)lds_pad;
    SR_REQUIRE(false, "host-only build: no kernels");
#else
    if (sym) {
        if (pl->ids16)
            hipLaunchKernelGGL((fused_trans_kernel<true, true>), dim3((unsigned)grid), dim3(256), lds_pad, st, a);
        else
            hipLaunchKernelGGL((fused_trans_kernel<false, true>), dim3((unsigned)grid), dim3(256), lds_pad, st, a);
    } else if (pl->ids16) {
        hipLaunchKernelGGL((fused_trans_kernel<true, false>), dim3((unsigned)grid), dim3(256), lds_pad, st, a);
    } else {
        hipLaunchKernelGGL((fused_trans_kernel<false, false>), dim3((unsigned)grid), dim3(256), lds_pad, st, a);
    }
#endif
    SR_HIP(hipGetLastError());
    return SIMRANK_OK;
}

int launch_fused_trans(const simrank_graph* g, const float* X, int64_t x_rows_pad, int64_t L, float* Y,
                       int64_t y_rows_pad, hipStream_t st, const int32_t* first_block) {
    SR_REQUIRE(g->fused, "graph has no fused plan");
    SR_REQUIRE(aligned16(X) && aligned16(Y), "fused leg needs 16-byte aligned operands");
    SR_REQUIRE(x_rows_pad >= g->n_cols && (x_rows_pad + 1) * 128 < (int64_t(1) << 31) && x_rows_pad < (int64_t(1) << 24) - 1,
               "fused leg: operand of %lld rows per panel", (long long)x_rows_pad);
    FusedArgs a{};
    a.X = X; a.Y = Y;
    a.x_rows_pad = x_rows_pad; a.y_rows_pad = y_rows_pad;
    a.L = L;
    a.x_panel_stride = x_rows_pad * 32;
    a.x_pitch = 128;
    a.x_bytes = int32_t(x_rows_pad * 128);
    a.x_sentinel = (int32_t)x_rows_pad;
    a.first_block = first_block;
    return launch_fused(g, a, st);
}

void fused_leg1_counts(const simrank_graph* g, int64_t L, const int32_t* first_block_host, int64_t* units, int64_t* skipped) {
    *units = *skipped = 0;
    const simrank_fused_plan* pl = g->fused;
    if (!pl) return;
    const int64_t n_panels = (L + 31) / 32;
    *units = n_panels * pl->n_units;
    if (!first_block_host) return;
    for (int64_t p = 0; p < n_panels; ++p)
        *skipped += std::lower_bound(pl->unit_last.begin(), pl->unit_last.end(), first_block_host[p]) - pl->unit_last.begin();
}

bool fused_sym_applies(const simrank_graph* g, int64_t x_rows_pad, int64_t L, int64_t y_rows_pad) {
    const simrank_fused_plan* pl = g->fused;
    if (!pl || !g->tun.fuse || g->tun.fuse_sym == 0 || g->tun.dense_terms != 3) return false;
    if (L != g->n_rows || g->n_cols > g->tun.fuse_max_rows) return false;
    if ((x_rows_pad + 1) * 128 >= (int64_t(1) << 31) || (y_rows_pad + 1) * 128 >= (int64_t(1) << 31) ||
        x_rows_pad >= (int64_t(1) << 24) - 1 || y_rows_pad >= (int64_t(1) << 24) - 1)
        return false;
    if (g->tun.fuse_sym < 0) return 2 * pl->nnz_covered >= g->nnz;
    return true;
}

int launch_fused_sym(const simrank_graph* g, const float* X, int64_t x_rows_pad, int64_t L, float* Y, int64_t y_rows_pad,
                     float coef, float lbd, double eps, const uint8_t* ev, const float* ap, const float* prev,
                     unsigned long long* n_changed, int32_t set_diag, int32_t count_any, hipStream_t st) {
    SR_REQUIRE(fused_sym_applies(g, x_rows_pad, L, y_rows_pad), "fused leg 2 does not apply");
    SR_REQUIRE(aligned16(X) && aligned16(Y) && (!ap || aligned16(ap)) && (!prev || aligned16(prev)) &&
                   (!ev || reinterpret_cast<uintptr_t>(ev) % 4 == 0),
               "fused leg 2 needs 16-byte aligned operands");
    SR_REQUIRE(x_rows_pad >= g->n_cols && y_rows_pad >= g->n_rows && (!prev || n_changed), "fused leg 2: bad operands");
    FusedArgs a{};
    a.X = X; a.Y = Y;
    a.x_rows_pad = x_rows_pad; a.y_rows_pad = y_rows_pad;
    a.L = L;
    a.x_panel_stride = x_rows_pad * 32;
    a.x_pitch = 128;
    a.x_bytes = int32_t(x_rows_pad * 128);
    a.x_sentinel = (int32_t)x_rows_pad;
    a.coef = coef; a.lbd = lbd; a.eps = eps;
    a.ev = ev; a.ap = ap; a.prev = prev;
    a.n_changed = n_changed;
    a.set_diag = set_diag; a.count_any = count_any;
    return launch_fused(g, a, st, true);
}

bool fused_rowmajor_fits(const simrank_graph* g, const float* X, int64_t ldx, int64_t L, const float* Y, int64_t t_block,
                         int64_t t_pad) {
    const int64_t K = g->n_cols, M = g->n_rows;
    const int64_t tb = (t_block <= 0 || t_block > M) ? M : t_block;
    return g->fused && aligned16(X) && aligned16(Y) && ldx % 4 == 0 && ldx * 4 < (int64_t(1) << 24) && ldx >= 32 &&
           (K + 1) * ldx * 4 < (int64_t(1) << 32) && K < (int64_t(1) << 24) - 1 && L > 0 &&
           (tb % kFB == 0 || tb == M) && (tb + t_pad) % 4 == 0 && (M - (M - 1) / tb * tb + t_pad) % 4 == 0;
}

int launch_fused_trans_rowmajor(const simrank_graph* g, const float* X, int64_t ldx, int64_t L, float* Y, int64_t t_block,
                                int64_t t_pad, hipStream_t st) {
    SR_REQUIRE(fused_rowmajor_fits(g, X, ldx, L, Y, t_block, t_pad), "fused leg: row-major operand does not fit");
    FusedArgs a{};
    a.X = X; a.Y = Y;
    a.L = L;
    a.x_panel_stride = 32;
    a.x_pitch = uint32_t(ldx * 4);
    a.x_bytes = int32_t(uint32_t((g->n_cols - 1) * ldx * 4 + L * 4));
    a.x_sentinel = (int32_t)g->n_cols;
    a.y_chunked = 1;
    a.t_block = (t_block <= 0 || t_block > g->n_rows) ? g->n_rows : t_block;
    a.t_pad = t_pad;
    return launch_fused(g, a, st);
}

}

using namespace simrank;

extern "C" {

#ifdef SIMRANK_FUSED_STAMPS
__attribute__((visibility("default"))) int simrank_read_fused_stamps(unsigned long long* out, int64_t n_wg) {
    SR_HIP(hipDeviceSynchronize());
    SR_HIP(hipMemcpyFromSymbol(out, HIP_SYMBOL(simrank::g_fst), size_t(std::min<int64_t>(n_wg, simrank::kFstCap)) * 8 * sizeof(unsigned long long)));
    return SIMRANK_OK;
}
#endif

int simrank_graph_fused_stats(const simrank_graph* g, int64_t* n_steps, int64_t* nnz_covered,
                              int64_t* nnz_remainder) {
    SR_REQUIRE(g, "graph is NULL");
    const simrank_fused_plan* pl = g->fused;
    if (n_steps) *n_steps = pl ? pl->n_steps : 0;
    if (nnz_covered) *nnz_covered = pl ? pl->nnz_covered : 0;
    if (nnz_remainder) *nnz_remainder = pl ? pl->r_nnz : g->nnz;
    return SIMRANK_OK;
}

}
```

### simrank_amd/csrc/plan.hip

```cpp
#include <algorithm>
#include <chrono>
#include <cstdlib>
#include <cstring>
#include <numeric>
#include <vector>

#include "loop.h"
#include "side.h"

struct simrank_plan {
    simrank::side_t s;
    unsigned long long* counters = nullptr;
    unsigned long long* host_counters[2] = {nullptr, nullptr};
    hipEvent_t counted[2] = {nullptr, nullptr};
    hipStream_t stream = nullptr;
    int32_t asym = 0;
    int32_t updates = 0;
    int32_t identity_leg1 = 1;
    int32_t at_identity = 0;
    std::vector<hipEvent_t> ev_pool;
    std::vector<hipEvent_t> ev_used;
    bool timing = false;
};

namespace simrank {

static int stamp(simrank_plan* p) {
    if (!p->timing || p->ev_pool.empty()) return SIMRANK_OK;
    hipEvent_t e = p->ev_pool.back();
    p->ev_pool.pop_back();
    p->ev_used.push_back(e);
    SR_HIP(hipEventRecord(e, p->stream));
    return SIMRANK_OK;
}

static int leg_pair(simrank_plan* p, double eps, int32_t exact_count, int slot) {
    const bool timed = p->timing && p->ev_pool.size() >= 3;
    const bool from_identity = p->at_identity && p->identity_leg1;
    p->at_identity = 0;
    const int rc = side_leg_pair(p->s, p->s, from_identity, p->asym != 0, eps, exact_count, p->counters, p->host_counters[slot],
                                 p->stream, [&] { return timed ? stamp(p) : SIMRANK_OK; });
    if (rc) return rc;
    SR_HIP(hipEventRecord(p->counted[slot], p->stream));
    return SIMRANK_OK;
}

static int read_count(simrank_plan* p, int slot, unsigned long long* sum) {
    SR_HIP(hipEventSynchronize(p->counted[slot]));
    unsigned long long t = 0;
    for (int i = 0; i < SIMRANK_CHANGED_SLOTS; ++i) t += p->host_counters[slot][i];
    *sum = t;
    return SIMRANK_OK;
}

}

using namespace simrank;

extern "C" {

int simrank_plan_destroy(simrank_plan* p) {
    if (!p) return SIMRANK_OK;
    if (p->stream) (void)hipStreamSynchronize(p->stream);
    (void)pool_free(p->counters);
    for (int i = 0; i < 2; ++i) {
        if (p->host_counters[i]) (void)hipHostFree(p->host_counters[i]);
        if (p->counted[i]) (void)hipEventDestroy(p->counted[i]);
    }
    for (hipEvent_t e : p->ev_pool) (void)hipEventDestroy(e);
    for (hipEvent_t e : p->ev_used) (void)hipEventDestroy(e);
    side_free(p->s);
    delete p;
    return SIMRANK_OK;
}

int simrank_plan_create(int64_t n, int64_t nnz, const int32_t* rowptr, const int32_t* col, const float* rowscale,
                        const simrank_plan_options* opt, void* stream, simrank_plan** out) {
    SR_REQUIRE(out, "out is NULL");
    *out = nullptr;
    const bool timed = std::getenv("SIMRANK_TIME_BUILD") != nullptr;
    const auto t_start = std::chrono::steady_clock::now();
    auto lap = [&](const char* what) {
        if (timed)
            std::fprintf(stderr, "simrank_plan_create: %6.1f ms  %s\n",
                         std::chrono::duration<double, std::milli>(std::chrono::steady_clock::now() - t_start).count(), what);
    };
    PlanPrep pp;
    int rc = plan_prepare(n, nnz, rowptr, col, rowscale, opt, &pp);
    if (rc) return rc;
    lap("validated, ordered, renamed");
    simrank_plan* p = new simrank_plan;
    side_t& a = p->s;
    side_shape(a, n, n, opt->storage_fp16 != 0);
    p->stream = as_stream(stream);
    a.coef = opt->coef;
    a.lbd = opt->lbd;
    p->asym = pp.asym ? 1 : 0;
    if (const char* e = std::getenv("SIMRANK_IDENTITY_LEG1")) p->identity_leg1 = (*e == '0') ? 0 : 1;
    auto fail = [&](int code) { simrank_plan_destroy(p); return code; };
    {
        Tuning t = tuning_snapshot();
        if (p->s.half) {
            t.fuse_unit = int64_t(1) << 20;
            if (t.fuse_min == 3) {
                t.fuse_min = 4;
                if (t.fuse_group == 3) t.fuse_group = 4;
            } else if (t.fuse_min == 0 && t.fuse_pays < 0) {
                t.fuse_pays = 256;
                if (t.fuse_group == 3) t.fuse_group = 4;
            }
        }
        if (t.fuse == 1 && ((t.triangle && n >= 64) || p->asym) &&
            (p->s.half || ((opt->dense_terms == 0 || opt->dense_terms == 3) && n <= t.fuse_max_rows &&
                         (p->s.rows_pad + 1) * 128 < (int64_t(1) << 31))))
            t.dense_lazy = 1;
        std::function<int(simrank_graph*)> counts = [&](simrank_graph* g) -> int {
            if (!opt->evidence) return SIMRANK_OK;
            const int rce = side_evidence_alloc(a, 0, p->stream);
            return rce ? rce : simrank_evidence_counts_blocked(g, 0, n, a.ev, a.rows_pad, p->stream);
        };
        rc = graph_create_with(t, n, n, nnz, pp.rp.data(), pp.cl.data(), pp.rs.data(), &a.g, &counts);
    }
    if (rc) return fail(rc);
    lap("graph object (evidence counts queued)");
    if (opt->dense_terms == 1) {
        rc = simrank_graph_set_dense_terms(p->s.g, 1);
        if (rc) return fail(rc);
    }
    if (p->s.half && !p->s.g->fused) {
        set_error("storage_fp16 needs the one-launch plan (tuning fuse = 1) and a graph that has one");
        return fail(SIMRANK_ERR_INVALID);
    }
    auto counters = [&]() -> int {
        SIDE_HIP(pool_hip_alloc((void**)&p->counters, sizeof(unsigned long long) * SIMRANK_CHANGED_SLOTS));
        for (int i = 0; i < 2; ++i) {
            SIDE_HIP(hipHostMalloc((void**)&p->host_counters[i], sizeof(unsigned long long) * SIMRANK_CHANGED_SLOTS, hipHostMallocPortable));
            SIDE_HIP(hipEventCreateWithFlags(&p->counted[i], hipEventDisableTiming));
        }
        return SIMRANK_OK;
    };
    rc = counters();
    if (!rc) rc = side_alloc(a, pp.ord, pp.inv, p->stream);
    if (!rc && !a.half) {
        auto table = [&]() -> int {
            const size_t bytes = pp.first_block.size() * sizeof(int32_t);
            SIDE_HIP(pool_hip_alloc((void**)&a.first_block, bytes));
            SIDE_HIP(hipMemcpyAsync(a.first_block, pp.first_block.data(), bytes, hipMemcpyHostToDevice, p->stream));
            SIDE_HIP(hipStreamSynchronize(p->stream));
            a.first_block_host = pp.first_block;
            return SIMRANK_OK;
        };
        rc = table();
    }
    if (rc) return fail(rc);
    lap("matrices allocated, orders uploaded, stream drained");
    if (opt->evidence) rc = side_restrict(a, p->stream);
    if (!rc && opt->apriori) rc = side_prior(a, opt->apriori, opt->ld_apriori, p->stream);
    if (rc) return fail(rc);
    lap("live segments, prior");
    rc = simrank_plan_reset(p);
    if (rc) return fail(rc);
    lap("reset queued");
    *out = p;
    return SIMRANK_OK;
}

int simrank_plan_reset(simrank_plan* p) {
    SR_REQUIRE(p, "plan is NULL");
    SR_REQUIRE(p->s.S[0], "the plan's matrices were released (simrank_plan_trim)");
    p->updates = 0;
    p->at_identity = 1;
    return side_reset(p->s, p->stream);
}

int simrank_plan_step(simrank_plan* p, double eps, int32_t exact_count, int64_t* n_changed) {
    SR_REQUIRE(p, "plan is NULL");
    SR_REQUIRE(p->s.S[0], "the plan's matrices were released (simrank_plan_trim)");
    const int rc = leg_pair(p, eps, exact_count, 0);
    if (rc) return rc;
    p->s.cur ^= 1;
    ++p->updates;
    if (n_changed) {
        unsigned long long c = 0;
        const int rc2 = read_count(p, 0, &c);
        if (rc2) return rc2;
        *n_changed = (int64_t)c;
    }
    return SIMRANK_OK;
}

int simrank_plan_run_cb(simrank_plan* p, int32_t iterations, double eps, simrank_progress_fn progress, void* user,
                        int32_t* updates_done, int32_t* converged_at) {
    SR_REQUIRE(p, "plan is NULL");
    SR_REQUIRE(iterations >= 0, "iterations < 0");
    SR_REQUIRE(p->s.S[0], "the plan's matrices were released (simrank_plan_trim)");
    const int rc = simrank_plan_reset(p);
    if (rc) return rc;
    struct {
        simrank_plan* p;
        double eps;
        int queue(int slot) { return leg_pair(p, eps, 0, slot); }
        int count(int slot, bool* zero) {
            unsigned long long c = 0;
            const int rcc = read_count(p, slot, &c);
            *zero = c == 0;
            return rcc;
        }
        void adopt() { p->s.cur ^= 1; }
        int drop() { return SIMRANK_OK; }
    } ops{p, eps};
    const LoopResult r = run_loop(ops, iterations, eps, p->s.n < kSpeculateBelow, progress, user);
    if (r.rc) return r.rc;
    SR_HIP(hipStreamSynchronize(p->stream));
    p->updates = r.done;
    if (updates_done) *updates_done = r.done;
    if (converged_at) *converged_at = r.conv;
    return SIMRANK_OK;
}

int simrank_plan_run(simrank_plan* p, int32_t iterations, double eps, int32_t* updates_done, int32_t* converged_at) {
    return simrank_plan_run_cb(p, iterations, eps, nullptr, nullptr, updates_done, converged_at);
}

int simrank_plan_result(simrank_plan* p, float* dst, int64_t ld) {
    SR_REQUIRE(p && dst && ld >= p->s.n, "bad result arguments");
    SR_REQUIRE(p->s.S[0], "the plan's matrices were released (simrank_plan_trim)");
    const side_t& a = p->s;
    const float* src = nullptr;
    float* wide = nullptr;
    int rc = side_f32(a, p->stream, &src, &wide);
    if (!rc) rc = simrank_permute_layout(src, 32, a.rows_pad, dst, ld, 0, a.n, a.n, a.inv, a.inv, 4, p->stream);
    if (wide) {
        (void)hipStreamSynchronize(p->stream);
        (void)pool_free(wide);
    }
    return rc;
}

int simrank_plan_result_f64(simrank_plan* p, double* dst, int64_t ld) {
    SR_REQUIRE(p && dst && ld >= p->s.n, "bad result arguments");
    SR_REQUIRE(p->s.S[0], "the plan's matrices were released (simrank_plan_trim)");
    return side_result_f64(p->s, dst, ld, p->stream);
}

int simrank_plan_evidence_u8(simrank_plan* p, uint8_t* dst, int64_t ld) {
    SR_REQUIRE(p && dst && ld >= p->s.n, "bad evidence arguments");
    SR_REQUIRE(p->s.ev, "the plan was created without evidence");
    return side_evidence_u8(p->s, dst, ld, p->stream, "simrank_plan_evidence_u8");
}

int simrank_plan_trim(simrank_plan* p) {
    SR_REQUIRE(p, "plan is NULL");
    if (p->stream) SR_HIP(hipStreamSynchronize(p->stream));
    side_trim(p->s);
    return SIMRANK_OK;
}

int simrank_plan_rows_f32(simrank_plan* p, const int32_t* rows, int32_t n_rows, float* dst, int64_t ld) {
    SR_REQUIRE(p && rows && dst && n_rows > 0 && ld >= p->s.n, "bad row arguments");
    SR_REQUIRE(p->s.S[0], "the plan's matrices were released (simrank_plan_trim)");
    return side_rows_f32(p->s, rows, n_rows, dst, ld, p->stream);
}

int simrank_plan_topk(simrank_plan* p, int32_t k, int32_t exclude_diag, int32_t* idx_host, float* val_host) {
    SR_REQUIRE(p && idx_host && val_host && k > 0 && k <= 1024, "bad top-k arguments");
    SR_REQUIRE(p->s.S[0], "the plan's matrices were released (simrank_plan_trim)");
    return side_topk(p->s, k, exclude_diag, idx_host, val_host, p->stream, "simrank_plan_topk");
}

int simrank_plan_set_timing(simrank_plan* p, int32_t updates) {
    SR_REQUIRE(p && updates >= 0 && updates <= (1 << 20), "bad timing arguments");
    for (hipEvent_t e : p->ev_used) p->ev_pool.push_back(e);
    p->ev_used.clear();
    while ((int64_t)p->ev_pool.size() < 3 * (int64_t)updates) {
        hipEvent_t e;
        SR_HIP(hipEventCreate(&e));
        p->ev_pool.push_back(e);
    }
    p->timing = updates > 0;
    return SIMRANK_OK;
}

int simrank_plan_leg_times(simrank_plan* p, double* leg1_ms, double* leg2_ms, int32_t* updates) {
    SR_REQUIRE(p, "plan is NULL");
    SR_HIP(hipStreamSynchronize(p->stream));
    double a = 0, b = 0;
    const size_t n = p->ev_used.size() / 3;
    for (size_t u = 0; u < n; ++u) {
        float t1 = 0, t2 = 0;
        SR_HIP(hipEventElapsedTime(&t1, p->ev_used[3 * u], p->ev_used[3 * u + 1]));
        SR_HIP(hipEventElapsedTime(&t2, p->ev_used[3 * u + 1], p->ev_used[3 * u + 2]));
        a += t1;
        b += t2;
    }
    if (leg1_ms) *leg1_ms = n ? a / (double)n : 0.0;
    if (leg2_ms) *leg2_ms = n ? b / (double)n : 0.0;
    if (updates) *updates = (int32_t)n;
    for (hipEvent_t e : p->ev_used) p->ev_pool.push_back(e);
    p->ev_used.clear();
    return SIMRANK_OK;
}

int simrank_plan_info(const simrank_plan* p, int64_t* n, int32_t* updates, const simrank_graph** graph) {
    SR_REQUIRE(p, "plan is NULL");
    if (n) *n = p->s.n;
// ... 12 lines not shown
```

### simrank_amd/csrc/planprep.hip

```cpp
#include <algorithm>
#include <atomic>
#include <cmath>
#include <numeric>
#include <thread>

#include "common.h"

namespace simrank {

static int check_csr(int64_t n_rows, int64_t n_cols, int64_t nnz, const int32_t* rowptr, const int32_t* col) {
    SR_REQUIRE(rowptr[0] == 0 && rowptr[n_rows] == nnz, "rowptr does not span [0, nnz]");
    for (int64_t a = 0; a < n_rows; ++a)
        SR_REQUIRE(rowptr[a + 1] >= rowptr[a] && rowptr[a + 1] <= nnz, "rowptr not monotone at row %lld", (long long)a);
    for (int64_t j = 0; j < nnz; ++j) SR_REQUIRE(col[j] >= 0 && col[j] < n_cols, "column index %d out of range", col[j]);
    return SIMRANK_OK;
}

static int check_prior(const float* a, int64_t ld, int64_t n, int which, bool half, bool* asym = nullptr) {
    if (!a) return SIMRANK_OK;
    SR_REQUIRE(ld >= n, "prior %d: ld %lld < n", which, (long long)ld);
    for (int64_t i = 0; i < n; ++i)
        for (int64_t j = i; j < n; ++j) {
            const float v = a[i * ld + j];
            if (j > i && !(v == a[j * ld + i])) {
                SR_REQUIRE(asym && !half, "this plan needs symmetric priors (prior %d, element %lld, %lld)", which, (long long)i,
                           (long long)j);
                *asym = true;
            }
            SR_REQUIRE(!half || (std::isfinite(v) && std::fabs(v) < 3.99f),
                       "storage_fp16 needs finite prior values below 4 in magnitude (element %lld, %lld)", (long long)i,
                       (long long)j);
        }
    return SIMRANK_OK;
}

bool prior_symmetric(const float* a, int64_t ld, int64_t n) {
    if (!a || ld < n) return true;
    for (int64_t i = 0; i < n; ++i)
        for (int64_t j = i + 1; j < n; ++j)
            if (!(a[i * ld + j] == a[j * ld + i])) return false;
    return true;
}

static int renamed(int64_t n_rows, const int32_t* rowptr, const int32_t* col, const float* scale,
                   const std::vector<int32_t>& ord, const std::vector<int32_t>& inv_cols, int64_t nnz, const char* what,
                   std::vector<int32_t>& rp, std::vector<int32_t>& cl, std::vector<float>& rs) {
    rp.assign((size_t)n_rows + 1, 0);
    cl.assign((size_t)std::max<int64_t>(1, nnz), 0);
    rs.assign((size_t)n_rows, 0.f);
    for (int64_t r = 0; r < n_rows; ++r) {
        const int32_t a = ord[(size_t)r];
        rp[(size_t)r + 1] = rp[(size_t)r] + (rowptr[a + 1] - rowptr[a]);
        rs[(size_t)r] = scale[a];
    }
    std::atomic<int64_t> dup_row{-1};
    auto work = [&](int64_t r0, int64_t r1) {
        for (int64_t r = r0; r < r1; ++r) {
            const int32_t a = ord[(size_t)r];
            const int32_t s = rowptr[a], e = rowptr[a + 1];
            int32_t* dst = cl.data() + rp[(size_t)r];
            for (int32_t j = s; j < e; ++j) dst[j - s] = inv_cols[(size_t)col[j]];
            std::sort(dst, dst + (e - s));
            for (int32_t j = 1; j < e - s; ++j)
                if (dst[j] == dst[j - 1]) {
                    int64_t seen = dup_row.load();
                    while ((seen < 0 || r < seen) && !dup_row.compare_exchange_weak(seen, r)) {}
                    break;
                }
        }
    };
    const int n_thr = nnz >= 100000 ? (int)std::max(8u, std::min(16u, std::thread::hardware_concurrency())) : 1;
    if (n_thr == 1) {
        work(0, n_rows);
    } else {
        std::vector<std::thread> th;
        int64_t r0 = 0;
        for (int t = 0; t < n_thr; ++t) {
            const int64_t target = nnz * (t + 1) / n_thr;
            int64_t r1 = t + 1 == n_thr ? n_rows
                                        : int64_t(std::upper_bound(rp.begin() + r0, rp.end(), (int32_t)target) - rp.begin()) - 1;
            r1 = std::max(r0, std::min(n_rows, r1));
            th.emplace_back(work, r0, r1);
            r0 = r1;
        }
        for (std::thread& x : th) x.join();
    }
    SR_REQUIRE(dup_row.load() < 0, "duplicate entry in row %d%s", ord[(size_t)dup_row.load()], what);
    return SIMRANK_OK;
}

static void length_order(int64_t n, const int32_t* rowptr, bool reorder, std::vector<int32_t>& ord, std::vector<int32_t>& inv) {
    ord.resize((size_t)n);
    inv.resize((size_t)n);
    std::iota(ord.begin(), ord.end(), 0);
    if (reorder)
        std::stable_sort(ord.begin(), ord.end(),
                         [rowptr](int32_t x, int32_t y) { return rowptr[x + 1] - rowptr[x] < rowptr[y + 1] - rowptr[y]; });
    for (int64_t r = 0; r < n; ++r) inv[(size_t)ord[(size_t)r]] = (int32_t)r;
}

static void refine_by_first_reference(int64_t n, const int32_t* rowptr, const int32_t* col, std::vector<int32_t>& ord,
                                      std::vector<int32_t>& inv) {
    std::vector<int32_t> first((size_t)n);
    for (int pass = 0; pass < 2; ++pass) {
        std::fill(first.begin(), first.end(), (int32_t)n);
        for (int64_t r = 0; r < n; ++r) {
            const int32_t a = ord[(size_t)r];
            for (int32_t j = rowptr[a]; j < rowptr[a + 1]; ++j)
                if (first[(size_t)col[j]] == (int32_t)n) first[(size_t)col[j]] = (int32_t)r;
        }
        std::stable_sort(ord.begin(), ord.end(), [&](int32_t x, int32_t y) {
            const int32_t lx = rowptr[x + 1] - rowptr[x], ly = rowptr[y + 1] - rowptr[y];
            return lx != ly ? lx < ly : first[(size_t)x] < first[(size_t)y];
        });
    }
    for (int64_t r = 0; r < n; ++r) inv[(size_t)ord[(size_t)r]] = (int32_t)r;
}

void first_block_table(int64_t n, const int32_t* rp, const int32_t* cl, std::vector<int32_t>& first_block) {
    std::vector<int32_t> first((size_t)n, kLeg1Never);
    for (int64_t a = 0; a < n; ++a)
        for (int32_t j = rp[a]; j < rp[a + 1]; ++j)
            if (first[(size_t)cl[j]] == kLeg1Never) first[(size_t)cl[j]] = (int32_t)a;
    first_block.assign((size_t)((n + 31) / 32), kLeg1Never);
    for (int64_t i = 0; i < n; ++i)
        if (first[(size_t)i] != kLeg1Never)
            first_block[(size_t)(i >> 5)] = std::min(first_block[(size_t)(i >> 5)], first[(size_t)i] / 128);
}

static void deal_order(int64_t n, int32_t deal, std::vector<int32_t>& ord, std::vector<int32_t>& inv) {
    if (deal <= 1 || n % (32 * int64_t(deal))) return;
    const int64_t unit = n % (128 * int64_t(deal)) == 0 ? 128 : 32, per = n / (unit * deal);
    std::vector<int32_t> dealt((size_t)n);
    for (int64_t b = 0; b < per; ++b)
        for (int64_t w = 0; w < deal; ++w)
            for (int64_t i = 0; i < unit; ++i)
                dealt[(size_t)((w * per + b) * unit + i)] = ord[(size_t)((b * deal + w) * unit + i)];
    ord.swap(dealt);
    for (int64_t r = 0; r < n; ++r) inv[(size_t)ord[(size_t)r]] = (int32_t)r;
}

int plan_prepare(int64_t n, int64_t nnz, const int32_t* rowptr, const int32_t* col, const float* rowscale,
                 const simrank_plan_options* opt, PlanPrep* out) {
    SR_REQUIRE(opt && rowptr && rowscale && (col || nnz == 0) && n > 0 && nnz >= 0 && out, "bad plan arguments");
    SR_REQUIRE(n < (int64_t(1) << 24) - 16, "a plan holds at most 2^24 nodes");
    SR_REQUIRE(opt->dense_terms == 0 || opt->dense_terms == 1 || opt->dense_terms == 3, "dense_terms must be 0, 1 or 3");
    int rc = check_csr(n, n, nnz, rowptr, col);
    out->asym = false;
    if (!rc) rc = check_prior(opt->apriori, opt->ld_apriori, n, 1, opt->storage_fp16 != 0, &out->asym);
    if (rc) return rc;
    length_order(n, rowptr, opt->reorder != 0, out->ord, out->inv);
    const Tuning t = tuning_snapshot();
    const bool refine = t.leg1_order > 0 || (t.leg1_order < 0 && n >= kSpeculateBelow);
    if (opt->reorder && refine && t.triangle && t.fuse == 1 && n >= 64 && !out->asym && !opt->storage_fp16)
        refine_by_first_reference(n, rowptr, col, out->ord, out->inv);
    rc = renamed(n, rowptr, col, rowscale, out->ord, out->inv, nnz, "", out->rp, out->cl, out->rs);
    if (!rc) first_block_table(n, out->rp.data(), out->cl.data(), out->first_block);
    return rc;
}

int shard_prepare(int64_t n, int64_t nnz, const int32_t* rowptr, const int32_t* col, const float* rowscale,
                  const float* apriori, int64_t ld_apriori, bool reorder, int32_t deal, PlanPrep* out, bool allow_asym) {
    SR_REQUIRE(rowptr && rowscale && (col || nnz == 0) && n > 0 && nnz >= 0 && out, "bad plan arguments");
    SR_REQUIRE(n < (int64_t(1) << 24) - 16, "a plan holds at most 2^24 nodes");
    int rc = check_csr(n, n, nnz, rowptr, col);
    out->asym = false;
    if (!rc) rc = check_prior(apriori, ld_apriori, n, 1, false, allow_asym ? &out->asym : nullptr);
    if (rc) return rc;
    length_order(n, rowptr, reorder, out->ord, out->inv);
    if (reorder) deal_order(n, deal, out->ord, out->inv);
    return renamed(n, rowptr, col, rowscale, out->ord, out->inv, nnz, "", out->rp, out->cl, out->rs);
}

int shard_biplan_prepare(int64_t n1, int64_t n2, int64_t nnz, const int32_t* rowptr12, const int32_t* col12,
                         const float* rowscale1, const float* rowscale2, const simrank_biplan_options* opt, int32_t deal1,
                         int32_t deal2, BiPlanPrep* out, bool allow_asym) {
    SR_REQUIRE(opt && rowptr12 && rowscale1 && rowscale2 && (col12 || nnz == 0) && n1 > 0 && n2 > 0 && nnz >= 0 && out,
               "bad plan arguments");
    SR_REQUIRE(n1 < (int64_t(1) << 24) - 16 && n2 < (int64_t(1) << 24) - 16, "a plan holds at most 2^24 nodes per group");
    int rc = check_csr(n1, n2, nnz, rowptr12, col12);
    out->asym = false;
    if (!rc) rc = check_prior(opt->apriori1, opt->ld_apriori1, n1, 1, false, allow_asym ? &out->asym : nullptr);
    if (!rc) rc = check_prior(opt->apriori2, opt->ld_apriori2, n2, 2, false, allow_asym ? &out->asym : nullptr);
    if (rc) return rc;
    std::vector<int32_t>& rowptr21 = out->rowptr21;
    std::vector<int32_t>& col21 = out->col21;
    rowptr21.assign((size_t)n2 + 1, 0);
    col21.assign((size_t)std::max<int64_t>(1, nnz), 0);
    for (int64_t j = 0; j < nnz; ++j) ++rowptr21[(size_t)col12[j] + 1];
    for (int64_t i = 0; i < n2; ++i) rowptr21[(size_t)i + 1] += rowptr21[(size_t)i];
    {
        std::vector<int32_t> fill(rowptr21.begin(), rowptr21.end() - 1);
        for (int64_t a = 0; a < n1; ++a)
            for (int32_t j = rowptr12[a]; j < rowptr12[a + 1]; ++j) col21[(size_t)fill[(size_t)col12[j]]++] = (int32_t)a;
    }
    const int64_t ns[2] = {n1, n2};
    const int32_t deals[2] = {deal1, deal2};
    const int32_t* rps[2] = {rowptr12, rowptr21.data()};
    const int32_t* cls[2] = {col12, col21.data()};
    const float* scales[2] = {rowscale1, rowscale2};
    for (int w = 0; w < 2; ++w) {
        length_order(ns[w], rps[w], opt->reorder != 0, out->ord[w], out->inv[w]);
        if (opt->reorder) deal_order(ns[w], deals[w], out->ord[w], out->inv[w]);
    }
    for (int w = 0; w < 2; ++w) {
        rc = renamed(ns[w], rps[w], cls[w], scales[w], out->ord[w], out->inv[w ^ 1], nnz, w ? " of group 2" : " of group 1",
                     out->rp[w], out->cl[w], out->rs[w]);
        if (rc) return rc;
    }
    return SIMRANK_OK;
}

int biplan_prepare(int64_t n1, int64_t n2, int64_t nnz, const int32_t* rowptr12, const int32_t* col12,
                   const float* rowscale1, const float* rowscale2, const simrank_biplan_options* opt, BiPlanPrep* out) {
    SR_REQUIRE(opt && rowptr12 && rowscale1 && rowscale2 && (col12 || nnz == 0) && n1 > 0 && n2 > 0 && nnz >= 0 && out,
               "bad plan arguments");
    SR_REQUIRE(n1 < (int64_t(1) << 24) - 16 && n2 < (int64_t(1) << 24) - 16, "a plan holds at most 2^24 nodes per group");
    int rc = check_csr(n1, n2, nnz, rowptr12, col12);
    out->asym = false;
    if (!rc) rc = check_prior(opt->apriori1, opt->ld_apriori1, n1, 1, false, &out->asym);
    if (!rc) rc = check_prior(opt->apriori2, opt->ld_apriori2, n2, 2, false, &out->asym);
    if (rc) return rc;
    std::vector<int32_t>& rowptr21 = out->rowptr21;
    std::vector<int32_t>& col21 = out->col21;
    rowptr21.assign((size_t)n2 + 1, 0);
    col21.assign((size_t)std::max<int64_t>(1, nnz), 0);
    for (int64_t j = 0; j < nnz; ++j) ++rowptr21[(size_t)col12[j] + 1];
    for (int64_t i = 0; i < n2; ++i) rowptr21[(size_t)i + 1] += rowptr21[(size_t)i];
    {
        std::vector<int32_t> fill(rowptr21.begin(), rowptr21.end() - 1);
        for (int64_t a = 0; a < n1; ++a)
            for (int32_t j = rowptr12[a]; j < rowptr12[a + 1]; ++j) col21[(size_t)fill[(size_t)col12[j]]++] = (int32_t)a;
    }
    const int64_t ns[2] = {n1, n2};
    const int32_t* rps[2] = {rowptr12, rowptr21.data()};
    const int32_t* cls[2] = {col12, col21.data()};
    const float* scales[2] = {rowscale1, rowscale2};
    for (int w = 0; w < 2; ++w) length_order(ns[w], rps[w], opt->reorder != 0, out->ord[w], out->inv[w]);
    for (int w = 0; w < 2; ++w) {
        rc = renamed(ns[w], rps[w], cls[w], scales[w], out->ord[w], out->inv[w ^ 1], nnz, w ? " of group 2" : " of group 1",
                     out->rp[w], out->cl[w], out->rs[w]);
        if (rc) return rc;
    }
    return SIMRANK_OK;
}

}
```

### simrank_amd/csrc/side.h

```cpp
#pragma once
#include <cstring>
#include <vector>

#include "common.h"

namespace simrank {

constexpr float kHalfScale = 16384.0f;

#define SIDE_HIP(call)                                                                            \
    do {                                                                                          \
        hipError_t e_ = (call);                                                                   \
        if (e_ != hipSuccess) {                                                                   \
            set_error("%s failed: %s (%s:%d)", #call, hipGetErrorString(e_), __FILE__, __LINE__); \
            (void)hipGetLastError();                                                              \
            return e_ == hipErrorOutOfMemory ? SIMRANK_ERR_ALLOC : SIMRANK_ERR_HIP;               \
        }                                                                                         \
    } while (0)

struct side_t {
    int64_t n = 0, k = 0, rows_pad = 0, k_rows_pad = 0;
    size_t mat_bytes = 0, t_bytes = 0;
    simrank_graph* g = nullptr;
    float* S[2] = {nullptr, nullptr};
    float* Tt = nullptr;
    uint8_t* ev = nullptr;
    float* prior = nullptr;
    int32_t* inv = nullptr;
    int32_t* ord_dev = nullptr;
    std::vector<int32_t> ord;
    float coef = 0.8f, lbd = 0.f;
    int32_t restrict_support = 0;
    int32_t half = 0;
    int cur = 0;
    int32_t* first_block = nullptr;
    std::vector<int32_t> first_block_host;
    int64_t leg1_units = 0, leg1_skipped = 0;
    int64_t dead_units = -1;
};

inline size_t side_f32_bytes(const side_t& a) { return size_t((a.n + 31) / 32) * size_t(a.rows_pad) * 32 * sizeof(float); }

inline void side_shape(side_t& a, int64_t n, int64_t k, bool half) {
    a.n = n;
    a.k = k;
    a.half = half ? 1 : 0;
    a.rows_pad = (n + 7) / 8 * 8 + 8;
    a.k_rows_pad = (k + 7) / 8 * 8 + 8;
    const size_t panels = half ? size_t((n + 63) / 64) : size_t((n + 31) / 32);
    a.mat_bytes = panels * size_t(a.rows_pad) * 128;
    a.t_bytes = panels * size_t(a.k_rows_pad) * 128;
}

inline int side_alloc(side_t& a, const std::vector<int32_t>& ord, const std::vector<int32_t>& inv, hipStream_t st) {
    const size_t ids = size_t(a.n) * sizeof(int32_t);
    for (float** b : {&a.S[0], &a.S[1]}) SIDE_HIP(pool_hip_alloc((void**)b, a.mat_bytes));
    SIDE_HIP(pool_hip_alloc((void**)&a.Tt, a.t_bytes));
    SIDE_HIP(pool_hip_alloc((void**)&a.inv, ids));
    SIDE_HIP(hipMemcpyAsync(a.inv, inv.data(), ids, hipMemcpyHostToDevice, st));
    a.ord = ord;
    SIDE_HIP(pool_hip_alloc((void**)&a.ord_dev, ids));
    SIDE_HIP(hipMemcpyAsync(a.ord_dev, a.ord.data(), ids, hipMemcpyHostToDevice, st));
    SIDE_HIP(hipStreamSynchronize(st));
    return SIMRANK_OK;
}

inline void side_trim(side_t& a) {
    (void)pool_free(a.S[0]); (void)pool_free(a.S[1]); (void)pool_free(a.Tt); (void)pool_free(a.prior);
    a.S[0] = a.S[1] = a.Tt = a.prior = nullptr;
}

inline void side_free(side_t& a) {
    side_trim(a);
    (void)pool_free(a.ev); (void)pool_free(a.inv); (void)pool_free(a.ord_dev); (void)pool_free(a.first_block);
    simrank_graph_destroy(a.g);
}

inline int side_reset(side_t& a, hipStream_t st) {
    a.cur = 0;
    if (a.half) return simrank_fill_identity_blocked_h16(a.S[0], a.n, a.n, a.rows_pad, 0, kHalfScale, st);
    return simrank_fill_identity_blocked(a.S[0], a.n, a.n, a.rows_pad, 0, st);
}

inline int side_evidence_alloc(side_t& a, int fill, hipStream_t st) {
    const size_t ev_bytes = size_t((a.n + 31) / 32) * size_t(a.rows_pad) * 32;
    hipError_t e = pool_hip_alloc((void**)&a.ev, ev_bytes);
    if (e == hipSuccess) e = hipMemsetAsync(a.ev, fill, ev_bytes, st);
    if (e != hipSuccess) {
        set_error("evidence counts: %s", hipGetErrorString(e));
        (void)hipGetLastError();
        return e == hipErrorOutOfMemory ? SIMRANK_ERR_ALLOC : SIMRANK_ERR_HIP;
    }
    return SIMRANK_OK;
}

inline int side_restrict(side_t& a, hipStream_t st) {
    int64_t live = 0, total = 1;
    const int rc = simrank_evidence_live_segments(a.ev, 32, a.rows_pad, a.n, a.n, &live, &total, st);
    if (rc) return rc;
    a.restrict_support = restrict_choice(a.g->tun, live, total);
    return SIMRANK_OK;
}

inline int side_prior(side_t& a, const float* apriori, int64_t ld_apriori, hipStream_t st) {
    const int64_t n = a.n;
    float* tmp = nullptr;
    SIDE_HIP(pool_hip_alloc((void**)&tmp, size_t(n) * size_t(n) * sizeof(float)));
    hipError_t e = pool_hip_alloc((void**)&a.prior, side_f32_bytes(a));
    if (e == hipSuccess) e = hipMemsetAsync(a.prior, 0, side_f32_bytes(a), st);
    if (e == hipSuccess) e = hipMemcpy2DAsync(tmp, size_t(n) * 4, apriori, size_t(ld_apriori) * 4, size_t(n) * 4, size_t(n),
                                              hipMemcpyHostToDevice, st);
    int rc = SIMRANK_OK;
    if (e == hipSuccess) {
        rc = simrank_permute_layout(tmp, n, 0, a.prior, 32, a.rows_pad, n, n, a.ord_dev, a.ord_dev, 4, st);
        e = hipStreamSynchronize(st);
    }
    (void)pool_free(tmp);
    if (e != hipSuccess) {
        set_error("plan prior upload: %s", hipGetErrorString(e));
        return SIMRANK_ERR_HIP;
    }
    return rc;
}

template <class Stamp>
int side_leg_pair(side_t& a, const side_t& o, bool from_identity, bool asym, double eps, int32_t exact_count,
                  unsigned long long* counters, unsigned long long* host_slot, hipStream_t st, Stamp&& stamp) {
    const int nx = a.cur ^ 1;
    simrank_epilogue ep{};
    ep.coef = a.coef;
    ep.lbd = a.lbd;
    ep.evidence = a.ev;
    ep.ld_evidence = 32;
    ep.apriori = a.prior;
    ep.ld_apriori = 32;
    ep.previous = a.S[a.cur];
    ep.ld_previous = 32;
    ep.eps = eps;
    ep.n_changed = counters;
    ep.diag_col0 = 0;
    ep.set_diag = 1;
    ep.symmetric = 1;
    ep.restrict_support = a.restrict_support;
    ep.count_any = exact_count ? 0 : 1;
    const int32_t* skip = nullptr;
    if (a.first_block && a.g->tun.leg1_skip && !from_identity && !asym && !a.half) {
        bool triangle = false;
        const int rct = spmm_blocked_is_triangle(a.g, a.Tt, a.k_rows_pad, a.n, a.S[nx], a.rows_pad, &ep, &triangle);
        if (rct) return rct;
        if (triangle) skip = a.first_block;
    }
    int rc = stamp();
    if (rc) return rc;
    bool skipping = false;
    rc = from_identity ? (a.half ? identity_leg1_blocked_h16(a.g, reinterpret_cast<uint16_t*>(a.Tt), a.k_rows_pad, kHalfScale, st)
                                 : identity_leg1_blocked(a.g, a.Tt, a.k_rows_pad, st))
         : a.half ? simrank_spmm_blocked_h16(a.g, o.S[o.cur], o.rows_pad, a.k, a.Tt, a.k_rows_pad, 1, nullptr, 0, kHalfScale, st)
                  : spmm_blocked_leg1(a.g, o.S[o.cur], o.rows_pad, a.k, a.Tt, a.k_rows_pad, skip, &skipping, st);
    a.leg1_units = a.leg1_skipped = 0;
    if (!rc && a.first_block && !from_identity && !a.half) {
        int64_t dead = 0;
        fused_leg1_counts(a.g, a.k, skipping ? a.first_block_host.data() : nullptr, &a.leg1_units, &dead);
        if (skipping) {
            if (a.dead_units < 0) a.dead_units = dead;
            a.leg1_skipped = a.dead_units;
        }
    }
    if (!rc) rc = stamp();
    if (rc) return rc;
    if (asym) {
        ep.symmetric = 0;
        ep.restrict_support = 0;
        rc = simrank_spmm_blocked(a.g, a.Tt, a.k_rows_pad, a.n, a.S[nx], a.rows_pad, 1, nullptr, st);
        if (!rc) rc = simrank_epilogue_apply_blocked(a.S[nx], a.S[nx], a.n, a.n, a.rows_pad, &ep, st);
    } else {
        rc = a.half ? simrank_spmm_blocked_h16(a.g, a.Tt, a.k_rows_pad, a.n, a.S[nx], a.rows_pad, 0, &ep, a.rows_pad, kHalfScale, st)
                    : simrank_spmm_blocked(a.g, a.Tt, a.k_rows_pad, a.n, a.S[nx], a.rows_pad, 0, &ep, st);
    }
    if (!rc) rc = stamp();
    if (rc) return rc;
    SR_HIP(hipMemcpyAsync(host_slot, counters, sizeof(unsigned long long) * SIMRANK_CHANGED_SLOTS, hipMemcpyDeviceToHost, st));
    return SIMRANK_OK;
}

inline int side_f32(const side_t& a, hipStream_t st, const float** src, float** scratch) {
    *src = a.S[a.cur];
    *scratch = nullptr;
    if (!a.half) return SIMRANK_OK;
    SR_HIP(pool_hip_alloc((void**)scratch, side_f32_bytes(a)));
    *src = *scratch;
    return simrank_widen_blocked_h16(a.S[a.cur], a.rows_pad, *scratch, a.rows_pad, a.n, a.n, kHalfScale, st);
}

inline int side_result_f64(const side_t& a, double* dst, int64_t ld, hipStream_t st) {
    const float* src = nullptr;
    float* wide = nullptr;
    int rc = side_f32(a, st, &src, &wide);
    if (!rc) rc = simrank_handback_f64(dst, ld, src, 32, a.rows_pad, a.n, a.inv, 0, st);
    (void)hipStreamSynchronize(st);
    (void)pool_free(wide);
    return rc;
}

inline int side_rows_f32(const side_t& a, const int32_t* rows, int32_t n_rows, float* dst, int64_t ld, hipStream_t st) {
    return rows_to_host(a.S[a.cur], a.rows_pad, a.n, a.inv, rows, n_rows, dst, ld, a.half ? 2 : 4, kHalfScale, st);
}

inline int side_evidence_u8(const side_t& a, uint8_t* dst, int64_t ld, hipStream_t st, const char* who) {
    uint8_t* tmp = nullptr;
    SR_HIP(pool_hip_alloc((void**)&tmp, size_t(a.n) * size_t(a.n)));
    const int rc = simrank_permute_layout(a.ev, 32, a.rows_pad, tmp, a.n, 0, a.n, a.n, a.inv, a.inv, 1, st);
    hipError_t e = hipSuccess;
    if (!rc) e = hipMemcpy2DAsync(dst, size_t(ld), tmp, size_t(a.n), size_t(a.n), size_t(a.n), hipMemcpyDeviceToHost, st);
    const hipError_t e2 = hipStreamSynchronize(st);
    (void)pool_free(tmp);
    if (e != hipSuccess || e2 != hipSuccess) {
        set_error("%s: %s", who, hipGetErrorString(e != hipSuccess ? e : e2));
        return SIMRANK_ERR_HIP;
    }
    return rc;
}

inline int side_topk(const side_t& a, int32_t k, int32_t exclude_diag, int32_t* idx_host, float* val_host, hipStream_t st,
                     const char* who) {
    const int64_t n = a.n;
    float* wide = nullptr;
    int32_t* idx_dev = nullptr;
    float* val_dev = nullptr;
    hipError_t e = hipSuccess;
    int rc = SIMRANK_OK;
    if (a.half) {
        e = pool_hip_alloc((void**)&wide, side_f32_bytes(a));
        if (e == hipSuccess) rc = simrank_widen_blocked_h16(a.S[a.cur], a.rows_pad, wide, a.rows_pad, n, n, kHalfScale, st);
    }
    if (e == hipSuccess) e = pool_hip_alloc((void**)&idx_dev, size_t(n) * size_t(k) * sizeof(int32_t));
    if (e == hipSuccess) e = pool_hip_alloc((void**)&val_dev, size_t(n) * size_t(k) * sizeof(float));
    std::vector<int32_t> idx_s;
    std::vector<float> val_s;
    if (e == hipSuccess && !rc) {
        rc = simrank_topk_rows_blocked(a.half ? wide : a.S[a.cur], a.rows_pad, n, n, 0, a.ord_dev, k, exclude_diag, idx_dev,
                                       val_dev, st);
        idx_s.resize(size_t(n) * size_t(k));
        val_s.resize(size_t(n) * size_t(k));
    }
    if (e == hipSuccess && !rc)
        e = hipMemcpyAsync(idx_s.data(), idx_dev, size_t(n) * size_t(k) * sizeof(int32_t), hipMemcpyDeviceToHost, st);
    if (e == hipSuccess && !rc)
        e = hipMemcpyAsync(val_s.data(), val_dev, size_t(n) * size_t(k) * sizeof(float), hipMemcpyDeviceToHost, st);
    if (e == hipSuccess) e = hipStreamSynchronize(st);
    else (void)hipStreamSynchronize(st);
    (void)pool_free(wide); (void)pool_free(idx_dev); (void)pool_free(val_dev);
    if (e != hipSuccess) {
        set_error("%s: %s", who, hipGetErrorString(e));
        (void)hipGetLastError();
        return SIMRANK_ERR_HIP;
    }
    if (rc) return rc;
    for (int64_t r = 0; r < n; ++r) {
        const int64_t node = a.ord[(size_t)r];
        std::memcpy(idx_host + node * k, idx_s.data() + r * k, size_t(k) * sizeof(int32_t));
        std::memcpy(val_host + node * k, val_s.data() + r * k, size_t(k) * sizeof(float));
    }
    return SIMRANK_OK;
}

inline int side_get(const side_t& a, const char* key, int64_t* value) {
    if (!strcmp(key, "restrict_support")) *value = a.restrict_support;
    else if (!strcmp(key, "iterate")) *value = (int64_t)(uintptr_t)a.S[a.cur];
    else if (!strcmp(key, "iterate_layout")) *value = a.half ? 2 : 0;
    else if (!strcmp(key, "iterate_stride")) *value = a.rows_pad;
    else if (!strcmp(key, "iterate_rows") || !strcmp(key, "iterate_col_hi")) *value = a.n;
    else if (!strcmp(key, "iterate_col_lo")) *value = 0;
    else if (!strcmp(key, "ids")) *value = (int64_t)(uintptr_t)a.ord_dev;
    else if (!strcmp(key, "leg1_units")) *value = a.leg1_units;
    else if (!strcmp(key, "leg1_skipped")) *value = a.leg1_skipped;
    else SR_REQUIRE(false, "unknown plan key '%s'", key);
    return SIMRANK_OK;
}

}
```

### simrank_amd/csrc/spmm.hip

```cpp
#include <algorithm>
#include <type_traits>

#include <mutex>

#include "common.h"

namespace simrank {

__device__ __forceinline__ int64_t imin(int64_t a, int64_t b) { return a < b ? a : b; }

__device__ __forceinline__ int64_t elem_at(int64_t r, int64_t c, int64_t ld, int64_t rows_pad) {
    return rows_pad ? ((c >> 5) * rows_pad + r) * 32 + (c & 31) : r * ld + c;
}

struct SpmmArgs {
    const int32_t* rowptr;
    const int32_t* col;
    const uint16_t* col16;
    int32_t blocked;
    int64_t x_rows_pad, y_rows_pad;
    int64_t x_span_bytes;
    int32_t x_sentinel;
    int32_t addr32;
    int32_t sh_rank, sh_mb;
// ... 1636 lines not shown
    int64_t I = (int64_t)((sqrt(8.0 * double(w) + 1.0) - 1.0) * 0.5);
    while (I * (I + 1) / 2 > w) --I;
    while ((I + 1) * (I + 2) / 2 <= w) ++I;
    const int64_t J = w - I * (I + 1) / 2;
    const int tid = threadIdx.x, r = tid >> 2, p = tid & 3;
    {
        const int64_t row = 64 * J + r, c = 64 * I + 16 * p;
        uint4 v = make_uint4(0u, 0u, 0u, 0u);
        if (row < n && c < n) {
            const uint8_t* src = cnt + elem_at(row, c, ld, rows_pad);
            if (vec16 && c + 16 <= n) {
                v = *reinterpret_cast<const uint4*>(src);
            } else {
                unsigned char b[16];
                for (int k = 0; k < 16; ++k) b[k] = c + k < n ? src[k] : 0;
                memcpy(&v, b, 16);
            }
        }
        *reinterpret_cast<uint4*>(&t[r][16 * p]) = v;
    }
    __syncthreads();
    const int64_t row = 64 * I + r, c = 64 * J + 16 * p;
    if (row >= n || c >= n) return;
    unsigned char b[16];
#pragma unroll
    for (int k = 0; k < 16; ++k) b[k] = t[16 * p + k][r];
    if (I == J)
#pragma unroll
        for (int k = 0; k < 16; ++k)
            if (16 * p + k >= r) b[k] = t[r][16 * p + k];
    uint8_t* dst = cnt + elem_at(row, c, ld, rows_pad);
    if (vec16 && c + 16 <= n) {
        uint4 v;
        memcpy(&v, b, 16);
        *reinterpret_cast<uint4*>(dst) = v;
    } else {
        for (int k = 0; k < 16; ++k)
            if (c + k < n) dst[k] = b[k];
    }
}

__global__ __launch_bounds__(256) void live_segments_kernel(const uint8_t* __restrict__ cnt, int64_t ld,
                                                            int64_t rows_pad, int64_t n_rows, int64_t n_cols,
                                                            unsigned long long* live) {
    const int64_t segs = (n_cols + 31) / 32;
    const int64_t total = n_rows * segs;
    unsigned mine = 0;
    if (rows_pad > 0 && (reinterpret_cast<uintptr_t>(cnt) & 15) == 0) {
        for (int64_t t = blockIdx.x * int64_t(blockDim.x) + threadIdx.x; t < total;
             t += int64_t(gridDim.x) * blockDim.x) {
            const int64_t sgm = t / n_rows, a = t - sgm * n_rows;
            const uint4* row = reinterpret_cast<const uint4*>(cnt + (sgm * rows_pad + a) * 32);
            const int n = int(imin(32, n_cols - sgm * 32));
            typedef unsigned v4u32 __attribute__((ext_vector_type(4)));
            const v4u32 lo = __builtin_nontemporal_load(reinterpret_cast<const v4u32*>(row));
            const v4u32 hi = __builtin_nontemporal_load(reinterpret_cast<const v4u32*>(row + 1));
            const unsigned w[8] = {lo.x, lo.y, lo.z, lo.w, hi.x, hi.y, hi.z, hi.w};
            unsigned any = 0;
#pragma unroll
            for (int k = 0; k < 8; ++k) {
                const int left = n - 4 * k;
                const unsigned mask = left >= 4 ? 0xFFFFFFFFu : left <= 0 ? 0u : (1u << (8 * left)) - 1u;
                any |= w[k] & mask;
            }
            mine += any ? 1u : 0u;
        }
    } else {
        for (int64_t t = blockIdx.x * int64_t(blockDim.x) + threadIdx.x; t < total;
             t += int64_t(gridDim.x) * blockDim.x) {
            const int64_t a = t / segs, sgm = t - a * segs;
            const uint8_t* row = cnt + elem_at(a, sgm * 32, ld, rows_pad);
            const int n = int(imin(32, n_cols - sgm * 32));
            unsigned any = 0;
            for (int c = 0; c < n; ++c) any |= row[c];
            mine += any ? 1u : 0u;
        }
    }
#pragma unroll
    for (int off = 32; off > 0; off >>= 1) mine += __shfl_down(mine, off);
    if ((threadIdx.x & 63) == 0 && mine) atomicAdd(live, (unsigned long long)mine);
}

__global__ __launch_bounds__(256) void shard_unpack_kernel(float* Y, int64_t ldy, const float* recv,
                                                           int64_t chunk, int rank, int mb, int64_t slot0) {
    const int h = blockIdx.y;
    if (h == rank) return;
    const int64_t slot = slot0 + blockIdx.x;
    int j = int((1.0 + sqrt(1.0 + 8.0 * double(slot))) * 0.5);
    while (int64_t(j) * (j - 1) / 2 > slot) --j;
    while (int64_t(j + 1) * j / 2 <= slot) ++j;
    const int i = int(slot - int64_t(j) * (j - 1) / 2);
    const float* src = recv + int64_t(h) * chunk + int64_t(blockIdx.x) * 1024;
    float* dst = Y + (int64_t(h) * mb + 32 * j) * ldy + 32 * i;
    const int c = threadIdx.x >> 3, r4 = (threadIdx.x & 7) * 4;
    *reinterpret_cast<float4*>(dst + c * ldy + r4) = *reinterpret_cast<const float4*>(src + c * 32 + r4);
}

}

using namespace simrank;

extern "C" {

int simrank_graph_create_counting(int64_t n_rows, int64_t n_cols, int64_t nnz, const int32_t* rowptr, const int32_t* col,
                                  const float* rowscale, int64_t col0, int64_t n_cols_ev, uint8_t* counts, int64_t ld,
                                  int64_t rows_pad, void* stream, simrank_graph** out) {
    SR_REQUIRE(counts && n_rows == n_cols, "evidence counts need a square pattern and a counts block");
    std::function<int(simrank_graph*)> hook = [&](simrank_graph* g) -> int {
        return rows_pad > 0 ? simrank_evidence_counts_blocked(g, col0, n_cols_ev, counts, rows_pad, stream)
                            : simrank_evidence_counts(g, col0, n_cols_ev, counts, ld, stream);
    };
    return graph_create_with(tuning_snapshot(), n_rows, n_cols, nnz, rowptr, col, rowscale, out, &hook);
}

int simrank_evidence_live_segments(const uint8_t* counts, int64_t ld, int64_t rows_pad, int64_t n_rows,
                                   int64_t n_cols, int64_t* live, int64_t* total, void* stream) {
    SR_REQUIRE(counts && live && total && n_rows > 0 && n_cols > 0 &&
                   (rows_pad ? rows_pad >= n_rows : ld >= n_cols), "bad evidence block");
    unsigned long long* d = nullptr;
    SR_HIP(hipMalloc((void**)&d, sizeof(unsigned long long)));
    hipStream_t st = as_stream(stream);
    hipError_t e = hipMemsetAsync(d, 0, sizeof(unsigned long long), st);
    unsigned long long h = 0;
    if (e == hipSuccess) {
        hipLaunchKernelGGL(live_segments_kernel, dim3(256 * 8), dim3(256), 0, st, counts, ld, rows_pad, n_rows,
                           n_cols, d);
        e = hipGetLastError();
    }
    if (e == hipSuccess) e = hipMemcpyAsync(&h, d, sizeof(h), hipMemcpyDeviceToHost, st);
    if (e == hipSuccess) e = hipStreamSynchronize(st);
    (void)hipFree(d);
    if (e != hipSuccess) {
        set_error("simrank_evidence_live_segments: %s", hipGetErrorString(e));
        return SIMRANK_ERR_HIP;
    }
    *live = (int64_t)h;
    *total = n_rows * ((n_cols + 31) / 32);
    return SIMRANK_OK;
}

int simrank_fill_identity(float* S, int64_t n_rows, int64_t n_cols, int64_t ld, int64_t col0,
                          void* stream) {
    SR_REQUIRE(S && n_rows > 0 && n_cols > 0 && ld >= n_cols, "bad identity block");
    const int64_t total = n_rows * n_cols;
    const int grid = (int)std::min<int64_t>((total + 255) / 256, 256 * 16);
    hipLaunchKernelGGL(fill_identity_kernel, dim3(grid), dim3(256), 0, as_stream(stream), S,
                       n_rows, n_cols, ld, col0);
    SR_HIP(hipGetLastError());
    return SIMRANK_OK;
}

struct Leg1Skip {
    bool dry = false, triangle = false, skipping = false;
    const int32_t* first_block = nullptr;
};

static int spmm_impl(const simrank_graph* g, const float* X, int64_t ldx, int64_t n_cols_x,
                     float* Y, int64_t ldy, int32_t transpose_out, int64_t t_block, int64_t t_pad,
                     const simrank_epilogue* ep, void* stream, bool blocked, int64_t x_rows_pad,
                     int64_t y_rows_pad, Leg1Skip* sk = nullptr) {
    SR_REQUIRE(t_pad >= 0 && t_pad < 4096, "t_pad out of range");
    SR_REQUIRE(g && X && Y, "NULL argument");
    const Tuning& T = g->tun;
    SR_REQUIRE(!(transpose_out && ep), "an epilogue needs transpose_out = 0");
    SpmmArgs a{};
    a.blocked = blocked ? 1 : 0;
    a.x_rows_pad = x_rows_pad;
    a.y_rows_pad = y_rows_pad;
    a.rowptr = g->rowptr;
    a.col = g->col;
    a.col16 = T.ids16 ? g->col16 : nullptr;
    a.rowscale = g->rowscale;
    a.huge_len = (int32_t)std::max<int64_t>(kHeavy, T.huge);
    a.has_huge = g->max_row_nnz >= a.huge_len ? 1 : 0;
    a.X = X;
    a.ldx = ldx;
    a.L = n_cols_x;
    a.Y = Y;
    a.ldy = ldy;
    a.M = g->n_rows;
    a.K = g->n_cols;
    a.tblock = (t_block <= 0 || t_block > g->n_rows) ? g->n_rows : t_block;
    a.tstride = (transpose_out && a.tblock == g->n_rows && ldy >= g->n_rows) ? ldy : 0;
    a.tpad = a.tstride ? 0 : t_pad;
    a.tvec = aligned16(Y) && (a.tstride ? a.tstride % 4 == 0
                                        : (a.tblock % 4 == 0 && a.tpad % 4 == 0 && g->n_rows % 4 == 0));
    a.xcd_map = (int)T.xcd_map;
    a.idx_mask = (int32_t)T.probe_mask;
    a.addr32 = (int32_t)T.addr32;
    a.probe = (int32_t)T.probe_flags;
    bool vec_ok = aligned16(X) && ldx % 4 == 0;
    if (!transpose_out) vec_ok = vec_ok && aligned16(Y) && ldy % 4 == 0;
    hipStream_t st = as_stream(stream);
    if (ep) {
        a.has_ep = 1;
        a.coef = ep->coef;
        a.lbd = ep->lbd;
        a.ev = ep->evidence;
        a.ld_ev = ep->ld_evidence;
        a.ap = ep->apriori;
        a.ld_ap = ep->ld_apriori;
        a.prev = ep->previous;
        a.ld_prev = ep->ld_previous;
        a.eps = ep->eps;
        a.n_changed = ep->n_changed;
        a.diag_col0 = ep->diag_col0;
        a.set_diag = ep->set_diag;
        a.restrict_support = ep->restrict_support;
        a.count_any = ep->count_any;
        if (blocked) a.ld_ev = a.ld_ap = a.ld_prev = 32;
        SR_REQUIRE(!a.ev || a.ld_ev >= n_cols_x || blocked, "evidence ld too small");
        SR_REQUIRE(!a.ap || a.ld_ap >= n_cols_x || blocked, "apriori ld too small");
        SR_REQUIRE(!a.prev || ((a.ld_prev >= n_cols_x || blocked) && a.n_changed),
                   "previous needs ld >= columns and a counter");
        if (a.ev) vec_ok = vec_ok && (reinterpret_cast<uintptr_t>(a.ev) % 4 == 0) && a.ld_ev % 4 == 0;
        if (a.ap) vec_ok = vec_ok && aligned16(a.ap) && a.ld_ap % 4 == 0;
        if (a.prev) vec_ok = vec_ok && aligned16(a.prev) && a.ld_prev % 4 == 0;
        if (a.prev && !(sk && sk->dry))
            SR_HIP(hipMemsetAsync(a.n_changed, 0, sizeof(unsigned long long) * SIMRANK_CHANGED_SLOTS, st));
    }
    int64_t panel = T.panel;
    if (panel == 0) panel = transpose_out ? 32 : 64;
    int64_t tile = T.tile;
    if (tile == 0) tile = 32;
    a.nt = (int32_t)T.stream_nt;
    const bool want_sym = ep && ep->symmetric && T.triangle && vec_ok && !transpose_out &&
                          n_cols_x == g->n_rows && ep->diag_col0 == 0 && g->n_rows >= 64;
    const bool one_launch_sym = blocked && want_sym && !transpose_out && ep && (!ep->restrict_support || T.fuse_sym > 0) &&
                                fused_sym_applies(g, x_rows_pad, n_cols_x, y_rows_pad);
    const simrank_dense_plan* dp = (vec_ok && T.dense_min > 0 && tile == 32) ? g->dense : nullptr;
    if (dp && want_sym) {
        const int64_t mode = T.dense_sym;
        if (mode == 0 || (mode < 0 && 2 * dp->nnz_covered < g->nnz)) dp = nullptr;
    }
    if (sk && sk->dry) {
        sk->triangle = blocked && want_sym && (one_launch_sym || !dp);
        return SIMRANK_OK;
    }
    if (blocked && transpose_out && g->fused && T.fuse && vec_ok && T.dense_terms == 3 && g->n_cols <= T.fuse_max_rows &&
        (x_rows_pad + 1) * 128 < (int64_t(1) << 31)) {
#ifdef SIMRANK_EXPERIMENT_FUSED2
        if (T.fuse == 2 && g->fused2 && (g->fused2->n_pslots == 0 || (n_cols_x + 31) / 32 <= g->fused2->cap_panels))
            return launch_fused2_trans(g, X, x_rows_pad, n_cols_x, Y, y_rows_pad, st);
#endif
        if (sk) sk->skipping = sk->first_block != nullptr;
        return launch_fused_trans(g, X, x_rows_pad, n_cols_x, Y, y_rows_pad, st, sk ? sk->first_block : nullptr);
    }
    if (!blocked && transpose_out && g->fused && T.fuse && T.fuse_shards && vec_ok && T.dense_terms == 3 &&
        g->n_cols <= T.fuse_max_rows) {
        const int64_t tb = a.tstride ? g->n_rows : t_block, tp = a.tstride ? a.tstride - g->n_rows : t_pad;
        if (fused_rowmajor_fits(g, X, ldx, n_cols_x, Y, tb, tp))
            return launch_fused_trans_rowmajor(g, X, ldx, n_cols_x, Y, tb, tp, st);
    }
    if (one_launch_sym)
        return launch_fused_sym(g, X, x_rows_pad, n_cols_x, Y, y_rows_pad, a.coef, a.lbd, a.eps, a.ev, a.ap, a.prev, a.n_changed,
                                a.set_diag, a.count_any, st);
    if (dp) {
        DenseUse use;
        const int rc = launch_dense_tiles(g, X, blocked ? -x_rows_pad : ldx, n_cols_x, want_sym, st, &use);
        if (rc) return rc;
        a.dpart = use.part;
        a.ldp = use.ldp;
        a.dslab0 = use.block_slab0;
        a.dnslab = use.block_nslab;
        a.rowptr = dp->r_rowptr;
        a.col = dp->r_col;
        a.col16 = T.ids16 ? dp->r_col16 : nullptr;
        a.has_huge = dp->r_max_row >= a.huge_len ? 1 : 0;
    }
    if (T.balance) {
        const int32_t* tr0 = dp ? dp->r_tile_row0 : g->tile_row0;
        if (tr0) {
            a.tile_row0 = tr0;
            a.n_tiles = dp ? dp->r_n_tiles : g->n_tiles;
            a.sym_map = dp ? dp->r_sym_map : g->sym_map;
            a.sym_blocks = dp ? dp->r_sym_blocks : g->sym_blocks;
        }
    }
    if (!vec_ok) {
        SR_REQUIRE(!blocked, "panel-blocked operands must be 16-byte aligned");
        return transpose_out ? launch_spmm<1, 32, kTrans, 32>(a, st)
                             : launch_spmm<1, 32, kPlain, 32>(a, st);
    }
    const bool lean_ok = T.lean && tile == 32 && ldx / 4 < (int64_t(1) << 24) &&
                         g->n_cols < (int64_t(1) << 24) && g->n_cols * (ldx / 4) < (int64_t(1) << 32) &&
                         g->n_rows < (int64_t(1) << 30);
    if (blocked) {
        SR_REQUIRE(lean_ok && (T.panel == 0 || T.panel == 32),
                   "panel-blocked operands need the lean kernel (tile 32, panel 32, < 2^24 rows)");
        if (want_sym) return launch_gather3<kSym>(a, st);
        return transpose_out ? launch_gather3<kTrans>(a, st) : launch_gather3<kPlain>(a, st);
    }
    if (lean_ok && want_sym) {
        a.tblock = g->n_rows;
        a.tstride = ldy;
        return launch_gather3<kSym>(a, st);
    }
    if (lean_ok && transpose_out && (T.panel == 0 || T.panel == 32))
        return launch_gather3<kTrans>(a, st);
    if (lean_ok && !transpose_out && (T.panel == 0 || T.panel == 32))
        return launch_gather3<kPlain>(a, st);
#define SR_TILE_SWITCH(LPR, TR)                                             \
    switch (tile) {                                                         \
        case 16: return launch_spmm<4, LPR, TR, 16>(a, st);                 \
        case 32: return launch_spmm<4, LPR, TR, 32>(a, st);                 \
        default: return launch_spmm<4, LPR, TR, 64>(a, st);                 \
    }
    if (want_sym) {
        a.tblock = g->n_rows;
        a.tstride = ldy;
        return launch_spmm<4, 8, kSym, 32>(a, st);
    }
    if (transpose_out) {
        if (panel > 64) panel = 64;
        if (panel == 64 && tile > 32) tile = 32;
        switch (panel) {
            case 16: SR_TILE_SWITCH(4, kTrans)
            case 32: SR_TILE_SWITCH(8, kTrans)
            default: SR_TILE_SWITCH(16, kTrans)
        }
    }
    switch (panel) {
        case 16: SR_TILE_SWITCH(4, kPlain)
        case 32: SR_TILE_SWITCH(8, kPlain)
        case 64: SR_TILE_SWITCH(16, kPlain)
        case 128: SR_TILE_SWITCH(32, kPlain)
        default: SR_TILE_SWITCH(64, kPlain)
    }
#undef SR_TILE_SWITCH
}

#ifdef SIMRANK_STAMPS
__attribute__((visibility("default"))) int simrank_read_stamps(unsigned long long* out16, int32_t reset) {
    SR_HIP(hipDeviceSynchronize());
    SR_HIP(hipMemcpyFromSymbol(out16, HIP_SYMBOL(simrank::g_stamps), 16 * sizeof(unsigned long long)));
    if (reset) {
        unsigned long long z[16] = {0};
        SR_HIP(hipMemcpyToSymbol(HIP_SYMBOL(simrank::g_stamps), z, sizeof(z)));
    }
    return SIMRANK_OK;
}
#endif

int simrank_fill_identity_blocked(float* S, int64_t n_rows, int64_t n_cols, int64_t rows_pad,
                                  int64_t col0, void* stream) {
    SR_REQUIRE(S && n_rows > 0 && n_cols > 0 && rows_pad >= n_rows, "bad identity block");
    const size_t bytes = size_t((n_cols + 31) / 32) * size_t(rows_pad) * 32 * sizeof(float);
    SR_HIP(hipMemsetAsync(S, 0, bytes, as_stream(stream)));
    const int grid = (int)std::min<int64_t>((n_cols + 255) / 256, 256 * 4);
    hipLaunchKernelGGL(set_diagonal_blocked_kernel, dim3(grid), dim3(256), 0, as_stream(stream), S, n_rows,
                       n_cols, rows_pad, col0);
    SR_HIP(hipGetLastError());
    return SIMRANK_OK;
}

}

__global__ __launch_bounds__(256) void identity_leg1_kernel(const int32_t* __restrict__ rowptr, const int32_t* __restrict__ col,
                                                            const float* __restrict__ rowscale, int64_t n_rows,
                                                            float* __restrict__ Tt, int64_t t_rows_pad) {
    const int lane = threadIdx.x & 63;
    const int64_t wave = (blockIdx.x * int64_t(blockDim.x) + threadIdx.x) >> 6;
    const int64_t nwaves = (int64_t(gridDim.x) * blockDim.x) >> 6;
    for (int64_t a = wave; a < n_rows; a += nwaves) {
        const float v = rowscale[a];
        float* base = Tt + ((a >> 5) * t_rows_pad) * 32 + (a & 31);
        for (int j = rowptr[a] + lane; j < rowptr[a + 1]; j += 64) base[int64_t(col[j]) * 32] = v;
    }
}

__global__ __launch_bounds__(256) void identity_leg1_h16_kernel(const int32_t* __restrict__ rowptr, const int32_t* __restrict__ col,
                                                                const float* __restrict__ rowscale, int64_t n_rows,
                                                                uint16_t* __restrict__ Tt, int64_t t_rows_pad, float scale) {
    const int lane = threadIdx.x & 63;
    const int64_t wave = (blockIdx.x * int64_t(blockDim.x) + threadIdx.x) >> 6;
    const int64_t nwaves = (int64_t(gridDim.x) * blockDim.x) >> 6;
    for (int64_t a = wave; a < n_rows; a += nwaves) {
        const uint16_t v = __builtin_bit_cast(uint16_t, _Float16(scale * rowscale[a]));
        uint16_t* base = Tt + ((a >> 6) * t_rows_pad) * 64 + (a & 63);
        for (int j = rowptr[a] + lane; j < rowptr[a + 1]; j += 64) base[int64_t(col[j]) * 64] = v;
    }
}

namespace simrank {
int identity_leg1_blocked_h16(const simrank_graph* g, uint16_t* Tt, int64_t t_rows_pad, float scale, void* stream) {
    SR_REQUIRE(g && Tt && t_rows_pad >= g->n_cols, "bad identity product");
    const size_t bytes = size_t((g->n_rows + 63) / 64) * size_t(t_rows_pad) * 64 * sizeof(uint16_t);
    SR_HIP(hipMemsetAsync(Tt, 0, bytes, as_stream(stream)));
    const int grid = (int)std::min<int64_t>((g->n_rows + 3) / 4, 256 * 8);
    hipLaunchKernelGGL(identity_leg1_h16_kernel, dim3(grid), dim3(256), 0, as_stream(stream), g->rowptr, g->col, g->rowscale,
                       g->n_rows, Tt, t_rows_pad, scale);
    SR_HIP(hipGetLastError());
    return SIMRANK_OK;
}

int identity_leg1_blocked(const simrank_graph* g, float* Tt, int64_t t_rows_pad, void* stream) {
    SR_REQUIRE(g && Tt && t_rows_pad >= g->n_cols, "bad identity product");
    const size_t bytes = size_t((g->n_rows + 31) / 32) * size_t(t_rows_pad) * 32 * sizeof(float);
    SR_HIP(hipMemsetAsync(Tt, 0, bytes, as_stream(stream)));
    const int grid = (int)std::min<int64_t>((g->n_rows + 3) / 4, 256 * 8);
    hipLaunchKernelGGL(identity_leg1_kernel, dim3(grid), dim3(256), 0, as_stream(stream), g->rowptr, g->col, g->rowscale,
                       g->n_rows, Tt, t_rows_pad);
    SR_HIP(hipGetLastError());
    return SIMRANK_OK;
}
}

extern "C" {

int simrank_spmm(const simrank_graph* g, const float* X, int64_t ldx, int64_t n_cols_x,
                 float* Y, int64_t ldy, int32_t transpose_out, int64_t t_block, int64_t t_pad,
                 const simrank_epilogue* ep, void* stream) {
    SR_REQUIRE(n_cols_x > 0 && ldx >= n_cols_x, "X: %lld columns, ld %lld", (long long)n_cols_x,
               (long long)ldx);
    SR_REQUIRE(transpose_out || ldy >= n_cols_x, "Y: ld %lld < %lld columns", (long long)ldy,
               (long long)n_cols_x);
    return spmm_impl(g, X, ldx, n_cols_x, Y, ldy, transpose_out, t_block, t_pad, ep, stream, false, 0, 0);
}

int simrank_spmm_blocked(const simrank_graph* g, const float* X, int64_t x_rows_pad, int64_t n_cols_x,
                         float* Y, int64_t y_rows_pad, int32_t transpose_out,
                         const simrank_epilogue* ep, void* stream) {
    SR_REQUIRE(g && n_cols_x > 0, "bad arguments");
    SR_REQUIRE(x_rows_pad >= g->n_cols && y_rows_pad >= (transpose_out ? n_cols_x : g->n_rows),
               "padded row counts %lld / %lld too small", (long long)x_rows_pad, (long long)y_rows_pad);
    return spmm_impl(g, X, 32, n_cols_x, Y, 32, transpose_out, 0, 0, ep, stream, true, x_rows_pad, y_rows_pad);
}

}

namespace simrank {
int spmm_blocked_is_triangle(const simrank_graph* g, const float* X, int64_t x_rows_pad, int64_t n_cols_x, float* Y,
                             int64_t y_rows_pad, const simrank_epilogue* ep, bool* triangle) {
    Leg1Skip sk;
    sk.dry = true;
    const int rc = spmm_impl(g, X, 32, n_cols_x, Y, 32, 0, 0, 0, ep, nullptr, true, x_rows_pad, y_rows_pad, &sk);
    *triangle = rc == SIMRANK_OK && sk.triangle;
    return rc;
}

int spmm_blocked_leg1(const simrank_graph* g, const float* X, int64_t x_rows_pad, int64_t n_cols_x, float* Y,
                      int64_t y_rows_pad, const int32_t* first_block, bool* skipping, void* stream) {
    Leg1Skip sk;
    sk.first_block = first_block;
    const int rc = spmm_impl(g, X, 32, n_cols_x, Y, 32, 1, 0, 0, nullptr, stream, true, x_rows_pad, y_rows_pad, &sk);
    *skipping = rc == SIMRANK_OK && sk.skipping;
    return rc;
}
}

extern "C" {

static int epilogue_apply_impl(const float* Q, int64_t ldq, float* Y, int64_t ldy, int64_t n_rows,
                               int64_t n_cols, const simrank_epilogue* ep, void* stream, int64_t rows_pad) {
    SR_REQUIRE(Q && Y && ep, "NULL argument");
    SR_REQUIRE(n_rows > 0 && n_cols > 0 && (rows_pad ? rows_pad >= n_rows : (ldq >= n_cols && ldy >= n_cols)),
               "bad block shape");
    SpmmArgs a{};
    a.y_rows_pad = rows_pad;
    a.has_ep = 1;
    a.coef = ep->coef;
    a.lbd = ep->lbd;
    a.ev = ep->evidence;
    a.ld_ev = ep->ld_evidence;
    a.ap = ep->apriori;
    a.ld_ap = ep->ld_apriori;
    a.prev = ep->previous;
    a.ld_prev = ep->ld_previous;
    a.eps = ep->eps;
    a.n_changed = ep->n_changed;
    a.diag_col0 = ep->diag_col0;
    a.set_diag = ep->set_diag;
    SR_REQUIRE(!a.prev || a.n_changed, "previous needs a counter");
    hipStream_t st = as_stream(stream);
    if (a.prev)
        SR_HIP(hipMemsetAsync(a.n_changed, 0, sizeof(unsigned long long) * SIMRANK_CHANGED_SLOTS, st));
    const int grid = (int)std::min<int64_t>((n_rows * n_cols + 255) / 256, 256 * 16);
    hipLaunchKernelGGL(epilogue_kernel, dim3(grid), dim3(256), 0, st, Q, ldq, Y, ldy, n_rows, n_cols, a);
    SR_HIP(hipGetLastError());
    return SIMRANK_OK;
}

static int spmm_shard_impl(const simrank_graph* g, const float* X, int64_t ldx, float* Y, int64_t ldy,
                           const simrank_epilogue* ep, int32_t rank, int32_t world, float* send,
                           int64_t chunk_floats, int32_t tile_lo, int32_t tile_hi, int32_t zero_counters,
                           void* stream) {
    SR_REQUIRE(g && X && Y && ep && send, "NULL argument");
    SR_REQUIRE(world >= 1 && rank >= 0 && rank < world && g->n_rows % (int64_t(world) * 32) == 0,
               "a symmetric sharded leg needs n_rows (%lld) divisible by 32 x world (%d)",
               (long long)g->n_rows, world);
    const int64_t mb = g->n_rows / world, tiles = mb / 32;
    SR_REQUIRE(tile_lo >= 0 && tile_lo < tile_hi && tile_hi <= tiles, "stage tiles [%d, %d) of %lld", tile_lo, tile_hi,
               (long long)tiles);
    const int64_t slot_lo = int64_t(tile_lo) * (tile_lo - 1) / 2, slot_hi = int64_t(tile_hi) * (tile_hi - 1) / 2;
    SR_REQUIRE(chunk_floats >= (slot_hi - slot_lo) * 1024 && (slot_hi == slot_lo || chunk_floats % 4 == 0),
               "send chunk too small or not a multiple of 4 floats");
    SR_REQUIRE(ep->diag_col0 == int64_t(rank) * mb && ldx >= mb && ldy >= mb && aligned16(X) && aligned16(Y) &&
                   aligned16(send) && ldx % 4 == 0 && ldy % 4 == 0, "bad shard operands");
    const Tuning& T = g->tun;
    SR_REQUIRE(T.lean && (T.tile == 0 || T.tile == 32) && (T.panel == 0 || T.panel == 32) &&
                   g->n_cols < (int64_t(1) << 24) && ldx / 4 < (int64_t(1) << 24) &&
                   g->n_cols * (ldx / 4) < (int64_t(1) << 32), "the symmetric sharded leg needs the lean kernel");
    SpmmArgs a{};
    a.rowptr = g->rowptr;
    a.col = g->col;
    a.col16 = T.ids16 ? g->col16 : nullptr;
    a.rowscale = g->rowscale;
    a.huge_len = (int32_t)std::max<int64_t>(kHeavy, T.huge);
    a.has_huge = g->max_row_nnz >= a.huge_len ? 1 : 0;
    a.X = X; a.ldx = ldx; a.L = mb; a.Y = Y; a.ldy = ldy;
    a.M = g->n_rows; a.K = g->n_cols;
    a.tblock = g->n_rows;
    a.xcd_map = (int)T.xcd_map;
    a.idx_mask = (int32_t)T.probe_mask;
    a.addr32 = (int32_t)T.addr32;
    a.probe = (int32_t)T.probe_flags;
    a.nt = 0;
    a.has_ep = 1;
    a.coef = ep->coef; a.lbd = ep->lbd;
    a.ev = ep->evidence; a.ld_ev = ep->ld_evidence;
    a.ap = ep->apriori; a.ld_ap = ep->ld_apriori;
    a.prev = ep->previous; a.ld_prev = ep->ld_previous;
    a.eps = ep->eps; a.n_changed = ep->n_changed;
    a.diag_col0 = ep->diag_col0; a.set_diag = ep->set_diag;
    a.restrict_support = ep->restrict_support;
    a.count_any = ep->count_any;
    SR_REQUIRE(!a.prev || a.n_changed, "previous needs a counter");
    SR_REQUIRE((!a.ev || (a.ld_ev % 4 == 0 && reinterpret_cast<uintptr_t>(a.ev) % 4 == 0)) &&
                   (!a.ap || (aligned16(a.ap) && a.ld_ap % 4 == 0)) &&
                   (!a.prev || (aligned16(a.prev) && a.ld_prev % 4 == 0)), "unaligned epilogue operand");
    a.sh_rank = rank; a.sh_mb = (int32_t)mb; a.sh_send = send; a.sh_chunk = chunk_floats;
    a.sh_tile0 = tile_lo; a.sh_ntiles = tile_hi - tile_lo; a.sh_slot0 = slot_lo;
    hipStream_t st = as_stream(stream);
    if (a.prev && zero_counters)
        SR_HIP(hipMemsetAsync(a.n_changed, 0, sizeof(unsigned long long) * SIMRANK_CHANGED_SLOTS, st));
    if (T.balance && g->tile_row0) {
        a.tile_row0 = g->tile_row0;
        a.n_tiles = g->n_tiles;
    }
    return launch_gather3<kShard>(a, st);
}

int simrank_spmm_shard(const simrank_graph* g, const float* X, int64_t ldx, float* Y, int64_t ldy,
                       const simrank_epilogue* ep, int32_t rank, int32_t world, float* send,
                       int64_t chunk_floats, void* stream) {
    SR_REQUIRE(g && world >= 1 && g->n_rows % (int64_t(world) * 32) == 0, "bad shard arguments");
    const int32_t tiles = (int32_t)(g->n_rows / world / 32);
    return spmm_shard_impl(g, X, ldx, Y, ldy, ep, rank, world, send, chunk_floats, 0, tiles, 1, stream);
}

int simrank_spmm_shard_stage(const simrank_graph* g, const float* X, int64_t ldx, float* Y, int64_t ldy,
                             const simrank_epilogue* ep, int32_t rank, int32_t world, float* send_stage,
                             int64_t stage_chunk_floats, int32_t tile_lo, int32_t tile_hi, int32_t zero_counters,
                             void* stream) {
    return spmm_shard_impl(g, X, ldx, Y, ldy, ep, rank, world, send_stage, stage_chunk_floats, tile_lo, tile_hi,
                           zero_counters, stream);
}

static int shard_unpack_impl(float* Y, int64_t ldy, const float* recv, int64_t chunk_floats, int32_t rank,
                             int32_t world, int64_t n_rows, int32_t tile_lo, int32_t tile_hi, void* stream) {
    SR_REQUIRE(Y && recv && world >= 1 && rank >= 0 && rank < world && n_rows % (int64_t(world) * 32) == 0,
               "bad shard unpack");
    const int mb = int(n_rows / world), tiles = mb / 32;
    SR_REQUIRE(tile_lo >= 0 && tile_lo < tile_hi && tile_hi <= tiles, "stage tiles [%d, %d) of %d", tile_lo, tile_hi, tiles);
    const int64_t slot_lo = int64_t(tile_lo) * (tile_lo - 1) / 2, slot_hi = int64_t(tile_hi) * (tile_hi - 1) / 2;
    const int64_t per_src = slot_hi - slot_lo;
    if (per_src == 0 || world == 1) return SIMRANK_OK;
    SR_REQUIRE(per_src < (int64_t(1) << 31), "too many tiles");
    SR_REQUIRE(ldy >= mb && ldy % 4 == 0 && aligned16(Y) && aligned16(recv) && chunk_floats % 4 == 0 &&
                   chunk_floats >= per_src * 1024, "bad shard unpack operands");
    hipLaunchKernelGGL(shard_unpack_kernel, dim3((unsigned)per_src, (unsigned)world), dim3(256), 0,
                       as_stream(stream), Y, ldy, recv, chunk_floats, (int)rank, mb, slot_lo);
    SR_HIP(hipGetLastError());
    return SIMRANK_OK;
}

int simrank_shard_unpack(float* Y, int64_t ldy, const float* recv, int64_t chunk_floats, int32_t rank,
                         int32_t world, int64_t n_rows, void* stream) {
    SR_REQUIRE(world >= 1 && n_rows % (int64_t(world) * 32) == 0, "bad shard unpack");
    return shard_unpack_impl(Y, ldy, recv, chunk_floats, rank, world, n_rows, 0, (int32_t)(n_rows / world / 32), stream);
}

int simrank_shard_unpack_stage(float* Y, int64_t ldy, const float* recv_stage, int64_t stage_chunk_floats,
                               int32_t rank, int32_t world, int64_t n_rows, int32_t tile_lo, int32_t tile_hi,
                               void* stream) {
    return shard_unpack_impl(Y, ldy, recv_stage, stage_chunk_floats, rank, world, n_rows, tile_lo, tile_hi, stream);
}

int simrank_epilogue_apply(const float* Q, int64_t ldq, float* Y, int64_t ldy, int64_t n_rows,
                           int64_t n_cols, const simrank_epilogue* ep, void* stream) {
    return epilogue_apply_impl(Q, ldq, Y, ldy, n_rows, n_cols, ep, stream, 0);
}

int simrank_epilogue_apply_blocked(const float* Q, float* Y, int64_t n_rows, int64_t n_cols,
                                   int64_t rows_pad, const simrank_epilogue* ep, void* stream) {
    return epilogue_apply_impl(Q, 32, Y, 32, n_rows, n_cols, ep, stream, rows_pad);
}
// ... 169 lines not shown
```

Before: 143.8.

## Compact leg-1 launch list, skip dead sub-blocks and unwritten output lines

Replaces the per-workgroup early-exit check for leg 1 with a host-built compacted launch list, so dead fused units are never launched at all. Each live entry also encodes the first live sub-block, so the kernel starts partway through its rounds. A per-panel line mask suppresses stores for output columns not yet live. This removes wasted workgroup launches, rounds and stores in the triangular leg, at the cost of extra device tables, more host preprocessing at plan time, and extra mask logic in the store path.

```diff
diff --git a/simrank_amd/csrc/api.hip b/simrank_amd/csrc/api.hip
--- a/simrank_amd/csrc/api.hip
+++ b/simrank_amd/csrc/api.hip
@@ -923,7 +923,7 @@
         SR_REQUIRE(value >= -1 && value <= 1, "restrict_support must be -1 (automatic), 0 or 1");
         t.restrict_support = value;
     } else if (!strcmp(key, "leg1_skip")) {
-        t.leg1_skip = value ? 1 : 0;
+        t.leg1_skip = value == 0 ? 0 : ((value > 0 && value <= 15 && (value & 1)) ? value : 1);
     } else if (!strcmp(key, "leg1_order")) {
         SR_REQUIRE(value >= -1 && value <= 1, "leg1_order must be -1 (by the graph's size), 0 or 1");
         t.leg1_order = value;
@@ -982,6 +982,8 @@
     SR_REQUIRE(g && key && value, "NULL argument");
     if (!strcmp(key, "fused_ids16")) *value = g->fused ? g->fused->ids16 : -1;
     else if (!strcmp(key, "gather_ids16")) *value = (g->col16 && g->tun.ids16) ? 1 : 0;
+    else if (!strcmp(key, "fused_n_units")) *value = g->fused ? g->fused->n_units : 0;
+    else if (!strcmp(key, "fused_units")) *value = g->fused ? (int64_t)(uintptr_t)g->fused->units : 0;
     else SR_REQUIRE(false, "unknown graph key '%s'", key);
     return SIMRANK_OK;
 }
diff --git a/simrank_amd/csrc/common.h b/simrank_amd/csrc/common.h
--- a/simrank_amd/csrc/common.h
+++ b/simrank_amd/csrc/common.h
@@ -127,9 +127,11 @@
     std::vector<float> rs;
     bool asym = false;
     std::vector<int32_t> first_block;
+    std::vector<int32_t> first_block_node;
 };
 constexpr int32_t kLeg1Never = 0x7FFFFFFF;
-void first_block_table(int64_t n, const int32_t* rp, const int32_t* cl, std::vector<int32_t>& first_block);
+void first_block_table(int64_t n, const int32_t* rp, const int32_t* cl, std::vector<int32_t>& first_block,
+                       std::vector<int32_t>* first_block_node = nullptr);
 struct BiPlanPrep {
     std::vector<int32_t> rowptr21, col21;
     std::vector<int32_t> ord[2], inv[2];
@@ -205,7 +207,7 @@
     int2* gmeta = nullptr;
     uint16_t* sids16 = nullptr;
     int32_t* sids32 = nullptr;
-    std::vector<int32_t> unit_last;
+    std::vector<int32_t> unit_b0, unit_nsub, unit_k;
 };
 
 #ifdef SIMRANK_EXPERIMENT_FUSED2
@@ -234,13 +236,25 @@
 constexpr int kSub = 4;
 void free_fused_plan(simrank_fused_plan* p);
 int build_fused_plan(simrank_graph* g, const int32_t* rowptr, const int32_t* col, const float* rowscale);
+constexpr int32_t kLeg1NoUnit = 0x3FFFFFFF;
+struct Leg1Live {
+    const int32_t* launch = nullptr;
+    int64_t grid = 0;
+    const uint32_t* line_mask = nullptr;
+};
+struct Leg1Launch {
+    std::vector<int32_t> launch;
+    std::vector<uint32_t> line_mask;
+    int64_t grid = 0, units = 0, dead = 0, launched = 0, lines_skipped = 0;
+};
+void build_leg1_launch(const simrank_fused_plan* pl, int64_t M, int64_t L, const int32_t* first_block,
+                       const int32_t* first_block_node, int64_t parts, Leg1Launch* out);
 int launch_fused_trans(const simrank_graph* g, const float* X, int64_t x_rows_pad, int64_t L, float* Y,
-                       int64_t y_rows_pad, hipStream_t st, const int32_t* first_block = nullptr);
-void fused_leg1_counts(const simrank_graph* g, int64_t L, const int32_t* first_block_host, int64_t* units, int64_t* skipped);
+                       int64_t y_rows_pad, hipStream_t st, const Leg1Live* live = nullptr);
 int spmm_blocked_is_triangle(const simrank_graph* g, const float* X, int64_t x_rows_pad, int64_t n_cols_x, float* Y,
                              int64_t y_rows_pad, const simrank_epilogue* ep, bool* triangle);
 int spmm_blocked_leg1(const simrank_graph* g, const float* X, int64_t x_rows_pad, int64_t n_cols_x, float* Y,
-                      int64_t y_rows_pad, const int32_t* first_block, bool* skipping, void* stream);
+                      int64_t y_rows_pad, const Leg1Live* live, bool* skipping, void* stream);
 bool fused_sym_applies(const simrank_graph* g, int64_t x_rows_pad, int64_t L, int64_t y_rows_pad);
 int launch_fused_sym(const simrank_graph* g, const float* X, int64_t x_rows_pad, int64_t L, float* Y, int64_t y_rows_pad,
                      float coef, float lbd, double eps, const uint8_t* ev, const float* ap, const float* prev,
diff --git a/simrank_amd/csrc/fused.hip b/simrank_amd/csrc/fused.hip
--- a/simrank_amd/csrc/fused.hip
+++ b/simrank_amd/csrc/fused.hip
@@ -61,7 +61,8 @@
     const float* prev;
     unsigned long long* n_changed;
     int32_t set_diag, count_any;
-    const int32_t* first_block;
+    const int32_t* launch;
+    const uint32_t* line_mask;
 };
 
 #ifndef SIMRANK_HOST_ONLY
@@ -104,7 +105,15 @@
 
     const int lane = threadIdx.x & 63;
     const int wave = __builtin_amdgcn_readfirstlane(threadIdx.x >> 6);
-    const uint32_t bid = blockIdx.x;
+    uint32_t bid = blockIdx.x;
+    int sb_first = 0;
+    if constexpr (!SYM) {
+        if (p.launch) {
+            const uint32_t e = uint32_t(p.launch[bid]);
+            bid = e & 0x3FFFFFFFu;
+            sb_first = int(e >> 30);
+        }
+    }
     const uint32_t local = bid >> 3;
     const int panel = int(local / uint32_t(p.n_units)) * 8 + int(bid & 7);
     if (panel >= p.n_panels) return;
@@ -124,9 +133,6 @@
     const int n_sub_all = un[8];
     const int n_sub_sym = SYM ? min(n_sub_all, int((c0 + 31) >> 7) - b0 + 1) : n_sub_all;
     if (SYM && n_sub_sym <= 0) return;
-    if constexpr (!SYM) {
-        if (p.first_block && b0 + n_sub_all - 1 < p.first_block[panel]) return;
-    }
     const int g = lane >> 3, q = lane & 7, gbase = lane & ~7;
     const uint32_t qoff = uint32_t(q) * 16u;
 
@@ -160,6 +166,7 @@
     const int round0 = wm[0];
     const int e1 = wm[1], e2 = wm[2], e3 = wm[3], e4 = wm[4];
     const int n_rounds = (p.probe & 1) ? 0 : (n_sub == 1 ? e1 : n_sub == 2 ? e2 : n_sub == 3 ? e3 : e4);
+    const int r_first = (SYM || (p.probe & 1) || sb_first == 0) ? 0 : (sb_first == 1 ? e1 : sb_first == 2 ? e2 : e3);
     auto fix_sid = [&](int v) -> int {
         if constexpr (IDS16) return v == 0xFFFF ? sent : (v & p.idx_mask);
         else return v < 0 ? sent : (v & p.idx_mask);
@@ -171,6 +178,14 @@
     };
     auto ld_sid = [&](int r) -> int { return fix_sid(ld_sid_raw(r)); };
     int iv0 = sent, iv1 = sent;
+    const uint32_t* lmp = nullptr;
+    uint32_t live_lines = 0xFFFFFFFFu;
+    if constexpr (!SYM) {
+        if (p.line_mask) {
+            lmp = p.line_mask + size_t(panel) * size_t((p.M + kFB - 1) / kFB) + b0;
+            live_lines = lmp[sb_first];
+        }
+    }
     {
         const int sbA = q >> 2, sbB = 2 + (q >> 2);
         const int2* src = p.gmeta + ((size_t(un[29]) * 4 + wave) * 8 + g) * 4 + (q & 3);
@@ -178,16 +193,16 @@
         int2 a = src[size_t(min(sbA, n_sub - 1)) * 4 * 8 * 4];
         int2 c = src[size_t(min(sbB, n_sub - 1)) * 4 * 8 * 4];
         int raw0 = 0, raw1 = 0;
-        if (n_rounds > 0) {
-            raw0 = ld_sid_raw(0);
-            raw1 = ld_sid_raw(1);
+        if (n_rounds > r_first) {
+            raw0 = ld_sid_raw(r_first);
+            raw1 = ld_sid_raw(r_first + 1);
         }
         __builtin_amdgcn_sched_barrier(0);
         if (sbA >= n_sub) a = make_int2(int(0xFFFFFFFFu), 0);
         if (sbB >= n_sub) c = make_int2(int(0xFFFFFFFFu), 0);
         dst[sbA * 4 * 8 * 4] = a;
         dst[sbB * 4 * 8 * 4] = c;
-        if (n_rounds > 0) {
+        if (n_rounds > r_first) {
             iv0 = fix_sid(raw0);
             iv1 = fix_sid(raw1);
         }
@@ -316,10 +331,10 @@
 
     FST(2);
     {
-        int sb = 0;
-        int r_base = 0;
+        int sb = sb_first;
+        int r_base = r_first;
         auto end_of = [&](int k) __attribute__((always_inline)) -> int { return k == 0 ? e1 : k == 1 ? e2 : k == 2 ? e3 : e4; };
-        int r_end = (p.probe & 1) ? 0 : e1;
+        int r_end = (p.probe & 1) ? 0 : end_of(sb_first);
         const int2* gmp = gm_lds + (wave * 8 + g) * 4;
         wave_lds_order();
         auto unpack = [](const int2& m) __attribute__((always_inline)) -> int3 {
@@ -327,7 +342,7 @@
             const int row = int(u & 255u), end = int(u >> 8);
             return make_int3(row == 255 ? -1 : row, m.y, end == 0xFFFFFF ? -1 : end);
         };
-        int3 m_cur = unpack(gmp[0]);
+        int3 m_cur = unpack(gmp[sb_first * 128]);
         float4 cur = make_float4(0.f, 0.f, 0.f, 0.f);
         int krow = 0;
         auto emit = [&](const int3& m, const float4& sv) __attribute__((always_inline)) {
@@ -521,13 +536,17 @@
                 const float* tw = tile + 32 * wave;
                 const __amdgpu_buffer_rsrc_t ysrd =
                     __builtin_amdgcn_make_buffer_rsrc(base, 0, (31 * cstride + 32) * 4, 0x00020000);
+                const uint32_t lines_out = live_lines & (cols_here >= 32 ? 0xFFFFFFFFu : (1u << cols_here) - 1u);
                 if ((rows_out & 3) == 0) {
 #pragma unroll
                     for (int it = 0; it < 4; ++it) {
                         const int x = lane + it * 64;
                         const int c = x >> 3;
                         const int r4 = (x & 7) * 4;
-                        if (c < cols_here && r4 < rows_out) {
+                        const uint32_t b8 = lines_out >> (8 * it);
+                        const uint32_t lo = (((b8 & 15u) * 0x00204081u) & 0x01010101u) * 255u;
+                        const uint32_t hi = ((((b8 >> 4) & 15u) * 0x00204081u) & 0x01010101u) * 255u;
+                        if (r4 < rows_out && __builtin_amdgcn_inverse_ballot_w64(uint64_t(hi) << 32 | lo)) {
                             const float4 v = *reinterpret_cast<const float4*>(tw + c * kTS + r4);
                             typedef unsigned v4u __attribute__((ext_vector_type(4)));
                             v4u o;
@@ -545,12 +564,15 @@
                 } else {
                     for (int x = lane; x < 32 * 32; x += 64) {
                         const int c = x >> 5, r = x & 31;
-                        if (c < cols_here && r < rows_out) base[c * cstride + r] = tw[c * kTS + r];
+                        if (r < rows_out && ((lines_out >> c) & 1u)) base[c * cstride + r] = tw[c * kTS + r];
                     }
                 }
             }
             ++sb;
             if (sb < n_sub) {
+                if constexpr (!SYM) {
+                    if (lmp) live_lines = lmp[sb];
+                }
                 __syncthreads();
                 r_base = r_end;
                 r_end = (p.probe & 1) ? 0 : end_of(sb);
@@ -572,10 +594,10 @@
             while (sb < n_sub && r + 1 == r_end) finish();
         };
         while (sb < n_sub && r_end == r_base) finish();
-        if (n_rounds > 0) {
+        if (n_rounds > r_first) {
             float4 vA[8], vB[8];
             issue8(iv0, vA);
-            int r = 0;
+            int r = r_first;
             while (r + 2 < n_rounds) {
                 const int iv2 = ld_sid(r + 2);
                 issue8(iv1, vB);
@@ -989,9 +1011,11 @@
     pl->nnz_covered = covered;
     pl->r_nnz = r_nnz;
     pl->ids16 = ids16 ? 1 : 0;
-    pl->unit_last.reserve(ulist.size());
-    for (const Unit& u : ulist) pl->unit_last.push_back(u.b0 + u.nsub - 1);
-    std::sort(pl->unit_last.begin(), pl->unit_last.end());
+    for (const Unit& u : ulist) {
+        pl->unit_b0.push_back(u.b0);
+        pl->unit_nsub.push_back(u.nsub);
+        pl->unit_k.push_back(u.k);
+    }
     dcols.resize(dcols.size() + 64, 0);
     abits.resize(abits.size() + 64 * 4, 0u);
     int rc = upload_vec(&pl->units, units);
@@ -1037,7 +1061,7 @@
     return SIMRANK_OK;
 }
 
-static int launch_fused(const simrank_graph* g, FusedArgs& a, hipStream_t st, bool sym = false) {
+static int launch_fused(const simrank_graph* g, FusedArgs& a, hipStream_t st, bool sym = false, int64_t list_grid = 0) {
     simrank_fused_plan* pl = g->fused;
     static std::mutex launch_mutex;
     std::lock_guard<std::mutex> launch_lock(launch_mutex);
@@ -1063,7 +1087,7 @@
     a.n_pslots = pl->n_pslots; a.n_cslots = pl->n_cslots;
     a.dcols16 = pl->dcols16; a.dcols32 = pl->dcols32; a.abits = pl->abits;
     a.gmeta = pl->gmeta; a.sids16 = pl->sids16; a.sids32 = pl->sids32;
-    const int64_t grid = int64_t((a.n_panels + 7) / 8) * 8 * a.n_units;
+    const int64_t grid = a.launch ? list_grid : int64_t((a.n_panels + 7) / 8) * 8 * a.n_units;
     SR_REQUIRE(grid > 0 && grid < (int64_t(1) << 31), "grid of %lld blocks", (long long)grid);
 #ifdef SIMRANK_FUSED_STAMPS
     static const unsigned lds_pad = getenv("SIMRANK_FUSED_PAD") ? (unsigned)atoi(getenv("SIMRANK_FUSED_PAD")) : 0u;
@@ -1095,7 +1119,7 @@
 }
 
 int launch_fused_trans(const simrank_graph* g, const float* X, int64_t x_rows_pad, int64_t L, float* Y,
-                       int64_t y_rows_pad, hipStream_t st, const int32_t* first_block) {
+                       int64_t y_rows_pad, hipStream_t st, const Leg1Live* live) {
     SR_REQUIRE(g->fused, "graph has no fused plan");
     SR_REQUIRE(aligned16(X) && aligned16(Y), "fused leg needs 16-byte aligned operands");
     SR_REQUIRE(x_rows_pad >= g->n_cols && (x_rows_pad + 1) * 128 < (int64_t(1) << 31) && x_rows_pad < (int64_t(1) << 24) - 1,
@@ -1108,19 +1132,70 @@
     a.x_pitch = 128;
     a.x_bytes = int32_t(x_rows_pad * 128);
     a.x_sentinel = (int32_t)x_rows_pad;
-    a.first_block = first_block;
-    return launch_fused(g, a, st);
-}
-
-void fused_leg1_counts(const simrank_graph* g, int64_t L, const int32_t* first_block_host, int64_t* units, int64_t* skipped) {
-    *units = *skipped = 0;
-    const simrank_fused_plan* pl = g->fused;
+    if (live) {
+        SR_REQUIRE(live->launch && live->grid > 0, "leg 1: launch list of %lld workgroups", (long long)live->grid);
+        a.launch = live->launch;
+        a.line_mask = live->line_mask;
+    }
+    return launch_fused(g, a, st, false, live ? live->grid : 0);
+}
+
+void build_leg1_launch(const simrank_fused_plan* pl, int64_t M, int64_t L, const int32_t* first_block,
+                       const int32_t* first_block_node, int64_t parts, Leg1Launch* out) {
+    *out = Leg1Launch();
     if (!pl) return;
-    const int64_t n_panels = (L + 31) / 32;
-    *units = n_panels * pl->n_units;
-    if (!first_block_host) return;
-    for (int64_t p = 0; p < n_panels; ++p)
-        *skipped += std::lower_bound(pl->unit_last.begin(), pl->unit_last.end(), first_block_host[p]) - pl->unit_last.begin();
+    const bool lines = !(parts & 2), compact = !(parts & 4), from_live = !(parts & 8);
+    const int64_t n_panels = (L + 31) / 32, n_units = pl->n_units, nblk = (M + kFB - 1) / kFB, tiles = (M + 31) / 32;
+    out->units = n_panels * n_units;
+    if (int64_t((n_panels + 7) / 8) * 8 * n_units >= kLeg1NoUnit) return;
+    std::vector<int32_t> per_xcd[8];
+    for (auto& v : per_xcd) v.reserve(size_t((n_panels + 7) / 8 * n_units));
+    out->line_mask.assign(size_t(n_panels) * size_t(nblk), 0u);
+    std::vector<int64_t> above(size_t(nblk) + 1);
+    for (int64_t P = 0; P < n_panels; ++P) {
+        std::vector<int32_t>& lst = per_xcd[P & 7];
+        const int64_t cols = std::min<int64_t>(32, L - 32 * P);
+        const int64_t fb = std::min<int64_t>(first_block[P], nblk);
+        std::fill(above.begin(), above.end(), 0);
+        uint32_t* lm = out->line_mask.data() + size_t(P) * size_t(nblk);
+        for (int64_t c = 0; c < cols; ++c) {
+            const int64_t f = std::min<int64_t>(first_block_node[32 * P + c], nblk);
+            ++above[size_t(f)];
+            if (f < nblk) lm[f] |= 1u << c;
+        }
+        for (int64_t b = 1; b < nblk; ++b) lm[b] |= lm[b - 1];
+        for (int64_t b = nblk, run = 0; b >= 0; --b) {
+            const int64_t here = above[size_t(b)];
+            above[size_t(b)] = run;
+            run += here;
+        }
+        for (int64_t u = 0; u < n_units; ++u) {
+            const int64_t b0 = pl->unit_b0[size_t(u)], nsub = pl->unit_nsub[size_t(u)];
+            const bool dead = b0 + nsub - 1 < fb;
+            const int64_t sb0 = dead ? nsub : (from_live ? std::max<int64_t>(0, fb - b0) : 0);
+            if (dead) {
+                ++out->dead;
+                if (!compact) lst.push_back(kLeg1NoUnit);
+            } else {
+                ++out->launched;
+                lst.push_back((int32_t)(uint32_t(((P >> 3) * n_units + u) * 8 + (P & 7)) | uint32_t(sb0) << 30));
+            }
+            if (pl->unit_k[size_t(u)] != 0) continue;
+            for (int64_t sb = 0; sb < nsub; ++sb) {
+                const int64_t b = b0 + sb, t = std::min<int64_t>(4, tiles - 4 * b);
+                out->lines_skipped += t * (sb < sb0 ? cols : (lines ? above[size_t(b)] : 0));
+            }
+        }
+    }
+    if (!compact) out->launched = out->units;
+    size_t longest = 0;
+    for (const auto& v : per_xcd) longest = std::max(longest, v.size());
+    out->grid = int64_t(longest) * 8;
+    out->launch.assign(longest * 8, kLeg1NoUnit);
+    for (size_t w = 0; w < longest * 8; ++w) {
+        const std::vector<int32_t>& v = per_xcd[w & 7];
+        if ((w >> 3) < v.size()) out->launch[w] = v[w >> 3];
+    }
 }
 
 bool fused_sym_applies(const simrank_graph* g, int64_t x_rows_pad, int64_t L, int64_t y_rows_pad) {
diff --git a/simrank_amd/csrc/plan.hip b/simrank_amd/csrc/plan.hip
--- a/simrank_amd/csrc/plan.hip
+++ b/simrank_amd/csrc/plan.hip
@@ -143,14 +143,28 @@
     if (!rc) rc = side_alloc(a, pp.ord, pp.inv, p->stream);
     if (!rc && !a.half) {
         auto table = [&]() -> int {
-            const size_t bytes = pp.first_block.size() * sizeof(int32_t);
-            SIDE_HIP(pool_hip_alloc((void**)&a.first_block, bytes));
-            SIDE_HIP(hipMemcpyAsync(a.first_block, pp.first_block.data(), bytes, hipMemcpyHostToDevice, p->stream));
+            const simrank_fused_plan* pl = a.g->fused;
+            if (!pl) return SIMRANK_OK;
+            a.live_units = (n + 31) / 32 * pl->n_units;
+            const int64_t parts = a.g->tun.leg1_skip;
+            if (!parts || p->asym) return SIMRANK_OK;
+            Leg1Launch ll;
+            build_leg1_launch(pl, n, n, pp.first_block.data(), pp.first_block_node.data(), parts, &ll);
+            a.live_dead = ll.dead; a.live_launched = ll.launched; a.live_lines = ll.lines_skipped;
+            if (ll.grid <= 0) return SIMRANK_OK;
+            const size_t lb = ll.launch.size() * sizeof(int32_t), mb = ll.line_mask.size() * sizeof(uint32_t);
+            SIDE_HIP(pool_hip_alloc((void**)&a.leg1_launch, lb));
+            SIDE_HIP(pool_hip_alloc((void**)&a.line_mask, mb));
+            SIDE_HIP(hipMemcpyAsync(a.leg1_launch, ll.launch.data(), lb, hipMemcpyHostToDevice, p->stream));
+            SIDE_HIP(hipMemcpyAsync(a.line_mask, ll.line_mask.data(), mb, hipMemcpyHostToDevice, p->stream));
             SIDE_HIP(hipStreamSynchronize(p->stream));
-            a.first_block_host = pp.first_block;
+            a.live.launch = a.leg1_launch;
+            a.live.grid = ll.grid;
+            a.live.line_mask = (parts & 2) ? nullptr : a.line_mask;
             return SIMRANK_OK;
         };
         rc = table();
+        lap("leg 1's launch list and line table");
     }
     if (rc) return fail(rc);
     lap("matrices allocated, orders uploaded, stream drained");
diff --git a/simrank_amd/csrc/planprep.hip b/simrank_amd/csrc/planprep.hip
--- a/simrank_amd/csrc/planprep.hip
+++ b/simrank_amd/csrc/planprep.hip
@@ -117,15 +117,19 @@
     for (int64_t r = 0; r < n; ++r) inv[(size_t)ord[(size_t)r]] = (int32_t)r;
 }
 
-void first_block_table(int64_t n, const int32_t* rp, const int32_t* cl, std::vector<int32_t>& first_block) {
+void first_block_table(int64_t n, const int32_t* rp, const int32_t* cl, std::vector<int32_t>& first_block,
+                       std::vector<int32_t>* first_block_node) {
     std::vector<int32_t> first((size_t)n, kLeg1Never);
     for (int64_t a = 0; a < n; ++a)
         for (int32_t j = rp[a]; j < rp[a + 1]; ++j)
             if (first[(size_t)cl[j]] == kLeg1Never) first[(size_t)cl[j]] = (int32_t)a;
     first_block.assign((size_t)((n + 31) / 32), kLeg1Never);
+    if (first_block_node) first_block_node->assign((size_t)n, (int32_t)((n + 127) / 128));
     for (int64_t i = 0; i < n; ++i)
-        if (first[(size_t)i] != kLeg1Never)
+        if (first[(size_t)i] != kLeg1Never) {
             first_block[(size_t)(i >> 5)] = std::min(first_block[(size_t)(i >> 5)], first[(size_t)i] / 128);
+            if (first_block_node) (*first_block_node)[(size_t)i] = first[(size_t)i] / 128;
+        }
 }
 
 static void deal_order(int64_t n, int32_t deal, std::vector<int32_t>& ord, std::vector<int32_t>& inv) {
@@ -155,7 +159,7 @@
     if (opt->reorder && refine && t.triangle && t.fuse == 1 && n >= 64 && !out->asym && !opt->storage_fp16)
         refine_by_first_reference(n, rowptr, col, out->ord, out->inv);
     rc = renamed(n, rowptr, col, rowscale, out->ord, out->inv, nnz, "", out->rp, out->cl, out->rs);
-    if (!rc) first_block_table(n, out->rp.data(), out->cl.data(), out->first_block);
+    if (!rc) first_block_table(n, out->rp.data(), out->cl.data(), out->first_block, &out->first_block_node);
     return rc;
 }
 
diff --git a/simrank_amd/csrc/side.h b/simrank_amd/csrc/side.h
--- a/simrank_amd/csrc/side.h
+++ b/simrank_amd/csrc/side.h
@@ -33,10 +33,11 @@
     int32_t restrict_support = 0;
     int32_t half = 0;
     int cur = 0;
-    int32_t* first_block = nullptr;
-    std::vector<int32_t> first_block_host;
-    int64_t leg1_units = 0, leg1_skipped = 0;
-    int64_t dead_units = -1;
+    int32_t* leg1_launch = nullptr;
+    uint32_t* line_mask = nullptr;
+    Leg1Live live;
+    int64_t live_units = 0, live_dead = 0, live_launched = 0, live_lines = 0;
+    int64_t leg1_units = 0, leg1_skipped = 0, leg1_launched = 0, leg1_lines_skipped = 0;
 };
 
 inline size_t side_f32_bytes(const side_t& a) { return size_t((a.n + 31) / 32) * size_t(a.rows_pad) * 32 * sizeof(float); }
@@ -72,7 +73,8 @@
 
 inline void side_free(side_t& a) {
     side_trim(a);
-    (void)pool_free(a.ev); (void)pool_free(a.inv); (void)pool_free(a.ord_dev); (void)pool_free(a.first_block);
+    (void)pool_free(a.ev); (void)pool_free(a.inv); (void)pool_free(a.ord_dev);
+    (void)pool_free(a.leg1_launch); (void)pool_free(a.line_mask);
     simrank_graph_destroy(a.g);
 }
 
@@ -143,12 +145,12 @@
     ep.symmetric = 1;
     ep.restrict_support = a.restrict_support;
     ep.count_any = exact_count ? 0 : 1;
-    const int32_t* skip = nullptr;
-    if (a.first_block && a.g->tun.leg1_skip && !from_identity && !asym && !a.half) {
+    const Leg1Live* skip = nullptr;
+    if (a.live.launch && a.g->tun.leg1_skip && !from_identity && !asym && !a.half) {
         bool triangle = false;
         const int rct = spmm_blocked_is_triangle(a.g, a.Tt, a.k_rows_pad, a.n, a.S[nx], a.rows_pad, &ep, &triangle);
         if (rct) return rct;
-        if (triangle) skip = a.first_block;
+        if (triangle) skip = &a.live;
     }
     int rc = stamp();
     if (rc) return rc;
@@ -157,13 +159,13 @@
                                  : identity_leg1_blocked(a.g, a.Tt, a.k_rows_pad, st))
          : a.half ? simrank_spmm_blocked_h16(a.g, o.S[o.cur], o.rows_pad, a.k, a.Tt, a.k_rows_pad, 1, nullptr, 0, kHalfScale, st)
                   : spmm_blocked_leg1(a.g, o.S[o.cur], o.rows_pad, a.k, a.Tt, a.k_rows_pad, skip, &skipping, st);
-    a.leg1_units = a.leg1_skipped = 0;
-    if (!rc && a.first_block && !from_identity && !a.half) {
-        int64_t dead = 0;
-        fused_leg1_counts(a.g, a.k, skipping ? a.first_block_host.data() : nullptr, &a.leg1_units, &dead);
+    a.leg1_units = a.leg1_skipped = a.leg1_launched = a.leg1_lines_skipped = 0;
+    if (!rc && a.live_units && !from_identity && !a.half) {
+        a.leg1_units = a.leg1_launched = a.live_units;
         if (skipping) {
-            if (a.dead_units < 0) a.dead_units = dead;
-            a.leg1_skipped = a.dead_units;
+            a.leg1_skipped = a.live_dead;
+            a.leg1_launched = a.live_launched;
+            a.leg1_lines_skipped = a.live_lines;
         }
     }
     if (!rc) rc = stamp();
@@ -274,6 +276,10 @@
     else if (!strcmp(key, "ids")) *value = (int64_t)(uintptr_t)a.ord_dev;
     else if (!strcmp(key, "leg1_units")) *value = a.leg1_units;
     else if (!strcmp(key, "leg1_skipped")) *value = a.leg1_skipped;
+    else if (!strcmp(key, "leg1_launched")) *value = a.leg1_launched;
+    else if (!strcmp(key, "leg1_lines_skipped")) *value = a.leg1_lines_skipped;
+    else if (!strcmp(key, "transposed")) *value = (int64_t)(uintptr_t)a.Tt;
+    else if (!strcmp(key, "transposed_stride")) *value = a.k_rows_pad;
     else SR_REQUIRE(false, "unknown plan key '%s'", key);
     return SIMRANK_OK;
 }
diff --git a/simrank_amd/csrc/spmm.hip b/simrank_amd/csrc/spmm.hip
--- a/simrank_amd/csrc/spmm.hip
+++ b/simrank_amd/csrc/spmm.hip
@@ -1812,7 +1812,7 @@
 
 struct Leg1Skip {
     bool dry = false, triangle = false, skipping = false;
-    const int32_t* first_block = nullptr;
+    const Leg1Live* live = nullptr;
 };
 
 static int spmm_impl(const simrank_graph* g, const float* X, int64_t ldx, int64_t n_cols_x,
@@ -1903,8 +1903,8 @@
         if (T.fuse == 2 && g->fused2 && (g->fused2->n_pslots == 0 || (n_cols_x + 31) / 32 <= g->fused2->cap_panels))
             return launch_fused2_trans(g, X, x_rows_pad, n_cols_x, Y, y_rows_pad, st);
 #endif
-        if (sk) sk->skipping = sk->first_block != nullptr;
-        return launch_fused_trans(g, X, x_rows_pad, n_cols_x, Y, y_rows_pad, st, sk ? sk->first_block : nullptr);
+        if (sk) sk->skipping = sk->live != nullptr;
+        return launch_fused_trans(g, X, x_rows_pad, n_cols_x, Y, y_rows_pad, st, sk ? sk->live : nullptr);
     }
     if (!blocked && transpose_out && g->fused && T.fuse && T.fuse_shards && vec_ok && T.dense_terms == 3 &&
         g->n_cols <= T.fuse_max_rows) {
@@ -2100,9 +2100,9 @@
 }
 
 int spmm_blocked_leg1(const simrank_graph* g, const float* X, int64_t x_rows_pad, int64_t n_cols_x, float* Y,
-                      int64_t y_rows_pad, const int32_t* first_block, bool* skipping, void* stream) {
+                      int64_t y_rows_pad, const Leg1Live* live, bool* skipping, void* stream) {
     Leg1Skip sk;
-    sk.first_block = first_block;
+    sk.live = live;
     const int rc = spmm_impl(g, X, 32, n_cols_x, Y, 32, 1, 0, 0, nullptr, stream, true, x_rows_pad, y_rows_pad, &sk);
     *skipping = rc == SIMRANK_OK && sk.skipping;
     return rc;
```

New measurement: 147.2, median of 6. Within noise of the previous version (+2.4%).
